# IC3Net/IC3Net

Hardware: NVIDIA H100
Metric: agent-env-steps/sec (higher is better)
Workload: dtype f32

## Files before the change

ic3net_b200/_lib.py:

```python
import ctypes as C
import os

import torch

_HERE = os.path.dirname(os.path.abspath(__file__))
LIB_PATH = os.path.join(_HERE, "libic3net_b200.so")

MAX_AGENTS = 32
MAX_HEADS = 4
MAX_HEAD_DIM = 16
MAX_PASSES = 4
CELL_LSTM, CELL_TANH = 0, 1
LSTM_IMG_BYTES = 786432

ERR_EPISODE_DONE = 1
ERR_ROUTE_OVERRUN = 2
ERR_BAD_ACTION = 4
ERR_PIPELINE = 0x100
ERR_FP16_RANGE = 0x200

PP_MODES = {"mixed": 0, "cooperative": 1, "competitive": 2}

_p = C.c_void_p


class PPCfg(C.Structure):
    _fields_ = [("B", C.c_int32), ("N", C.c_int32), ("dim", C.c_int32), ("vision", C.c_int32),
                ("mode", C.c_int32), ("naction", C.c_int32), ("env_id0", C.c_uint32), ("enemy_comm", C.c_int32),
                ("seed", C.c_uint64)]


class PPState(C.Structure):
    _fields_ = [("loc", _p), ("reached", _p), ("done", _p), ("success", _p), ("episode", _p), ("tick", _p)]


class RolloutIO(C.Structure):
    _fields_ = [("t", C.c_int32), ("max_steps", C.c_int32), ("nheads", C.c_int32), ("hard_attn", C.c_int32),
                ("comm_action_one", C.c_int32), ("last", C.c_int32), ("action", _p), ("t_ep", _p), ("fresh", _p),
                ("comm_next", _p), ("alive_next", _p), ("rec_reward", _p), ("rec_episode_mask", _p),
                ("rec_mini_mask", _p), ("rec_alive", _p), ("stat_reward", _p), ("stat_comm", _p),
                ("stat_success", _p), ("stat_episodes", _p), ("stat_steps", _p), ("batch_size", C.c_int32),
                ("reserved0", C.c_int32), ("halted", _p), ("rec_valid", _p), ("snap_T", C.c_int32),
                ("reserved1", C.c_int32), ("snap_fresh", _p), ("snap_comm", _p), ("snap_alive", _p), ("snap_tep", _p),
                ("snap_pp_loc", _p), ("snap_tj_loc", _p), ("snap_tj_alive", _p), ("snap_tj_last_act", _p),
                ("snap_tj_route_id", _p), ("head_partial", _p), ("head_b", _p), ("head_value", _p), ("head_logp", _p),
                ("head_dim", C.c_int32 * MAX_HEADS)]


class TJCfg(C.Structure):
    _fields_ = [("B", C.c_int32), ("N", C.c_int32), ("vision", C.c_int32), ("h", C.c_int32), ("w", C.c_int32),
                ("G", C.c_int32), ("P", C.c_int32), ("Lmax", C.c_int32), ("outside_cls", C.c_int32),
                ("car_cls", C.c_int32), ("vocab", C.c_int32), ("npath", C.c_int32), ("spawn_thr", C.c_uint32),
                ("env_id0", C.c_uint32), ("seed", C.c_uint64), ("grid", _p), ("route_len", _p), ("route_cells", _p)]


class TJState(C.Structure):
    _fields_ = [("loc", _p), ("alive", _p), ("wait", _p), ("route_id", _p), ("route_pos", _p), ("last_act", _p),
                ("completed", _p), ("cars_in_sys", _p), ("has_failed", _p), ("tick", _p)]


class PolicyCfg(C.Structure):
    _fields_ = [("B", C.c_int32), ("N", C.c_int32), ("H", C.c_int32), ("O", C.c_int32), ("nheads", C.c_int32),
                ("head_dim", C.c_int32 * MAX_HEADS), ("hard_attn", C.c_int32), ("comm_avg", C.c_int32),
                ("comm_mask_zero", C.c_int32), ("env_id0", C.c_uint32), ("seed", C.c_uint64),
                ("obs_off", C.c_int32), ("obs_vocab", C.c_int32), ("obs_ncount", C.c_int32), ("cell", C.c_int32),
                ("passes", C.c_int32), ("x_tanh", C.c_int32), ("h_from_x", C.c_int32), ("reserved0", C.c_int32)]


class PolicyParams(C.Structure):
    _fields_ = [("encoder_w", _p), ("encoder_b", _p), ("c_w", _p), ("c_b", _p), ("w_ih", _p), ("w_hh", _p),
                ("b_ih", _p), ("b_hh", _p), ("value_w", _p), ("value_b", _p),
                ("head_w", _p * MAX_HEADS), ("head_b", _p * MAX_HEADS), ("c_w_pass", _p * MAX_PASSES),
                ("c_b_pass", _p * MAX_PASSES), ("f_w_pass", _p * MAX_PASSES), ("f_b_pass", _p * MAX_PASSES)]


class PolicyPacked(C.Structure):
    _fields_ = [("enc_wT", _p), ("enc_b", _p), ("c_wT", _p), ("c_b", _p), ("lstm_wT", _p), ("lstm_b", _p),
                ("head_w", _p), ("head_b", _p), ("lstm_img", _p), ("bias_cat", _p), ("f_wT", _p), ("f_b", _p), ("flags", _p)]


class PolicyIO(C.Structure):
    _fields_ = [("x", _p), ("h", _p), ("c", _p), ("comm_action", _p), ("alive", _p), ("fresh", _p), ("tick", _p),
                ("draws", _p), ("h_out", _p), ("c_out", _p), ("value", _p), ("logp", _p), ("action", _p),
                ("workspace", _p), ("err", _p), ("pp_env", _p), ("pp_state", _p), ("tj_env", _p), ("tj_state", _p),
                ("x_table", _p), ("defer_heads", C.c_int32), ("pass_index", C.c_int32)]


class BpttPlan(C.Structure):
    _fields_ = [("cfg", C.POINTER(PolicyCfg)), ("w", C.POINTER(PolicyPacked)), ("pp_env", C.POINTER(PPCfg)),
                ("tj_env", C.POINTER(TJCfg)), ("x_table", _p), ("value_coeff", C.c_float), ("entr", C.c_float),
                ("workspace", _p)]


class BpttStepIO(C.Structure):
    _fields_ = [("t", C.c_int32), ("reserved0", C.c_int32), ("h_prev", _p), ("c_prev", _p), ("h_new", _p), ("fresh", _p), ("comm", _p), ("alive", _p), ("cut", _p),
                ("pp_loc", _p), ("tj_loc", _p), ("tj_alive", _p), ("tj_last_act", _p), ("tj_route_id", _p),
                ("logp", _p), ("action", _p), ("value", _p), ("ret", _p), ("adv", _p), ("alive_post", _p),
                ("valid", _p), ("dh", _p), ("dc", _p), ("err", _p)]


_PTR = C.c_void_p
SYMBOLS = {
    "ic3_version": (C.c_char_p, []),
    "ic3_strerror": (C.c_char_p, [C.c_int]),
    "ic3_launch_count": (C.c_uint64, []),
    "ic3_pp_reset": (C.c_int, [C.POINTER(PPCfg), C.POINTER(PPState), _PTR, _PTR, _PTR]),
    "ic3_pp_step": (C.c_int, [C.POINTER(PPCfg), C.POINTER(PPState), _PTR, C.c_int32, _PTR, _PTR, _PTR,
                              C.POINTER(RolloutIO), _PTR]),
    "ic3_pp_obs": (C.c_int, [C.POINTER(PPCfg), C.POINTER(PPState), _PTR, _PTR]),
    "ic3_pp_obs_bounded": (C.c_int, [C.POINTER(PPCfg), C.POINTER(PPState), _PTR, _PTR]),
    "ic3_tj_reset": (C.c_int, [C.POINTER(TJCfg), C.POINTER(TJState), _PTR, _PTR, _PTR]),
    "ic3_tj_step": (C.c_int, [C.POINTER(TJCfg), C.POINTER(TJState), _PTR, C.c_int32, _PTR, _PTR, _PTR, _PTR,
                              C.POINTER(RolloutIO), _PTR]),
    "ic3_tj_obs": (C.c_int, [C.POINTER(TJCfg), C.POINTER(TJState), _PTR, _PTR]),
    "ic3_tj_obs_bounded": (C.c_int, [C.POINTER(TJCfg), C.POINTER(TJState), _PTR, _PTR]),
    "ic3_policy_pack": (C.c_int, [C.POINTER(PolicyCfg), C.POINTER(PolicyParams), C.POINTER(PolicyPacked), _PTR]),
    "ic3_encoder_dense": (C.c_int, [C.POINTER(PolicyCfg), C.POINTER(PolicyPacked), _PTR, _PTR, _PTR]),
    "ic3_pp_encoder_index": (C.c_int, [C.POINTER(PPCfg), C.POINTER(PPState), C.POINTER(PolicyCfg),
                                       C.POINTER(PolicyPacked), _PTR, _PTR]),
    "ic3_tj_encoder_index": (C.c_int, [C.POINTER(TJCfg), C.POINTER(TJState), C.POINTER(PolicyCfg),
                                       C.POINTER(PolicyPacked), _PTR, _PTR]),
    "ic3_pp_obs_encode": (C.c_int, [C.POINTER(PPCfg), C.POINTER(PPState), C.POINTER(PolicyCfg),
                                    C.POINTER(PolicyPacked), _PTR, _PTR, _PTR]),
    "ic3_tj_obs_encode": (C.c_int, [C.POINTER(TJCfg), C.POINTER(TJState), C.POINTER(PolicyCfg),
                                    C.POINTER(PolicyPacked), _PTR, _PTR, _PTR]),
    "ic3_pp_encoder_table":(C.c_int, [C.POINTER(PPCfg), C.POINTER(PolicyCfg), C.POINTER(PolicyPacked), _PTR, _PTR]),
    "ic3_tj_encoder_table": (C.c_int, [C.POINTER(TJCfg), C.POINTER(PolicyCfg), C.POINTER(PolicyPacked), _PTR, _PTR]),
    "ic3_policy_workspace_bytes": (C.c_uint64, [C.POINTER(PolicyCfg)]),
    "ic3_policy_step": (C.c_int, [C.POINTER(PolicyCfg), C.POINTER(PolicyPacked), C.POINTER(PolicyIO), _PTR]),
    "ic3_policy_partial_ptr": (C.c_void_p, [C.POINTER(PolicyCfg), _PTR]),
    "ic3_policy_step_profile": (C.c_int, [C.POINTER(PolicyCfg), C.POINTER(PolicyPacked), C.POINTER(PolicyIO), _PTR,
                                          C.POINTER(C.c_float)]),
    "ic3_sample_actions": (C.c_int, [C.POINTER(PolicyCfg), _PTR, _PTR, _PTR, _PTR, _PTR]),
    "ic3_returns_scan": (C.c_int, [C.c_int32, C.c_int32, C.c_int32, C.c_float, C.c_float, _PTR, _PTR, _PTR, _PTR,
                                   _PTR]),
    "ic3_bptt_workspace_bytes": (C.c_uint64, [C.POINTER(BpttPlan)]),
    "ic3_bptt_begin": (C.c_int, [C.POINTER(BpttPlan), C.c_float, _PTR]),
    "ic3_bptt_step": (C.c_int, [C.POINTER(BpttPlan), C.POINTER(BpttStepIO), _PTR]),
    "ic3_bptt_prepare": (C.c_int, [C.POINTER(BpttPlan), C.POINTER(BpttStepIO), _PTR]),
    "ic3_bptt_finish": (C.c_int, [C.POINTER(BpttPlan), C.POINTER(PolicyParams), C.POINTER(PolicyParams), _PTR, _PTR]),
    "ic3_stat_reduce": (C.c_int, [C.c_int32, C.c_int32, _PTR, _PTR, _PTR, _PTR, _PTR, _PTR, _PTR, _PTR]),
    "ic3_rmsprop_step": (C.c_int, [C.c_int64, C.c_float, C.c_float, C.c_float, C.c_float, _PTR, _PTR, _PTR, _PTR]),
}

_lib = None


def load():
    global _lib
    if _lib is not None:
        return _lib
    if not os.path.exists(LIB_PATH):
        raise RuntimeError("ic3net_b200: %s not found; run `python -m ic3net_b200.build` "
                           "(there is no CPU fallback)" % LIB_PATH)
    lib = C.CDLL(LIB_PATH)
    for name, (res, args) in SYMBOLS.items():
        fn = getattr(lib, name)
        fn.restype = res
        fn.argtypes = args
    _lib = lib
    return lib


def check(rc):
    if rc != 0:
        raise RuntimeError("ic3net_b200 call failed (%d): %s" % (rc, load().ic3_strerror(rc).decode()))


def ptr(t):
    if t is None:
        return None
    assert t.is_cuda and t.is_contiguous(), "ic3net_b200 needs contiguous CUDA tensors"
    return t.data_ptr()


_raw_stream = getattr(torch._C, "_cuda_getCurrentRawStream", None)


def stream():
    if _raw_stream is not None:
        return _raw_stream(torch.cuda.current_device())
    return torch.cuda.current_stream().cuda_stream


def require_cuda():
    if not torch.cuda.is_available():
        raise RuntimeError("ic3net_b200 runs on a CUDA device only (no CPU fallback)")
    load()


def launch_count():
    return int(load().ic3_launch_count())
```

ic3net_b200/csrc/policy_tc.cu:

```cuda
#include <algorithm>

#include "policy_tc_kernels.cuh"


constexpr int TC_TILE_PAD = 8;
constexpr size_t LSTM_SMEM_BYTES = NSTAGE_P * STAGE_BYTES + 256 + TC_H * HEAD_PAD * sizeof(float) + 4 * TC_H * sizeof(float);

static int ctas_beside_lstm(const void* kern, int threads, size_t smem, int* per_sm, int* nsm) {
  cudaFuncAttributes la, ka;
  cudaError_t e = cudaFuncGetAttributes(&la, lstm_tc_kernel);
  if (e == cudaSuccess) e = cudaFuncGetAttributes(&ka, kern);
  int dev = 0, regs = 0, smem_sm = 0, reserved = 0, thr_sm = 0, blk_sm = 0;
  if (e == cudaSuccess) e = cudaGetDevice(&dev);
  if (e == cudaSuccess) e = cudaDeviceGetAttribute(nsm, cudaDevAttrMultiProcessorCount, dev);
  if (e == cudaSuccess) e = cudaDeviceGetAttribute(&regs, cudaDevAttrMaxRegistersPerMultiprocessor, dev);
  if (e == cudaSuccess) e = cudaDeviceGetAttribute(&smem_sm, cudaDevAttrMaxSharedMemoryPerMultiprocessor, dev);
  if (e == cudaSuccess) e = cudaDeviceGetAttribute(&reserved, cudaDevAttrReservedSharedMemoryPerBlock, dev);
  if (e == cudaSuccess) e = cudaDeviceGetAttribute(&thr_sm, cudaDevAttrMaxThreadsPerMultiProcessor, dev);
  if (e == cudaSuccess) e = cudaDeviceGetAttribute(&blk_sm, cudaDevAttrMaxBlocksPerMultiprocessor, dev);
  if (e != cudaSuccess) return (int)e;
  auto cta_regs = [](const cudaFuncAttributes& a, int nthr) { return ((a.numRegs * 32 + 255) / 256 * 256) * ((nthr + 31) / 32); };
  const long free_regs = (long)regs - cta_regs(la, TC_P_THREADS);
  const long free_smem = (long)smem_sm - (long)(LSTM_SMEM_BYTES + la.sharedSizeBytes + reserved);
  long n = free_regs / cta_regs(ka, threads);
  n = std::min(n, free_smem / (long)(smem + ka.sharedSizeBytes + reserved));
  n = std::min(n, (long)(thr_sm - TC_P_THREADS) / threads);
  n = std::min(n, (long)blk_sm - 1);
  *per_sm = n > 1 ? (int)n : 1;
  return IC3_OK;
}

int ic3_grid_beside_lstm(const void* kern, int threads, size_t smem, int nwork, int* grid) {
  struct Entry { const void* kern; int threads; size_t smem; int ctas; };
  static Entry cache[8];
  static int ncache = 0;
  int ctas = 0;
  for (int i = 0; i < ncache; ++i)
    if (cache[i].kern == kern && cache[i].threads == threads && cache[i].smem == smem) ctas = cache[i].ctas;
  if (ctas == 0) {
    cudaError_t e = cudaFuncSetAttribute(kern, cudaFuncAttributePreferredSharedMemoryCarveout, cudaSharedmemCarveoutMaxShared);
    if (e != cudaSuccess) return (int)e;
    int per_sm = 0, nsm = 0;
    const int rc = ctas_beside_lstm(kern, threads, smem, &per_sm, &nsm);
    if (rc) return rc;
    ctas = per_sm * nsm;
    if (ncache < 8) cache[ncache++] = Entry{kern, threads, smem, ctas};
  }
  *grid = nwork < ctas ? nwork : ctas;
  return IC3_OK;
}

static int launch_lstm(const ic3_policy_cfg* cfg, const ic3_policy_io* io, const ic3_policy_packed* w, const __half* a_img,
                       int ntiles_pad, size_t smem, int nout, float* partial, cudaStream_t s) {
  static int max_ctas = 0;
  auto kern = lstm_tc_kernel;
  if (max_ctas == 0) {
    cudaError_t e = cudaFuncSetAttribute(kern, cudaFuncAttributeMaxDynamicSharedMemorySize, (int)smem);
    if (e != cudaSuccess) return (int)e;
    int per_sm = 0, dev = 0, nsm = 0;
    e = cudaOccupancyMaxActiveBlocksPerMultiprocessor(&per_sm, kern, TC_P_THREADS, smem);
    if (e == cudaSuccess) e = cudaGetDevice(&dev);
    if (e == cudaSuccess) e = cudaDeviceGetAttribute(&nsm, cudaDevAttrMultiProcessorCount, dev);
    if (e != cudaSuccess || per_sm <= 0) return e != cudaSuccess ? (int)e : IC3_E_RANGE;
    max_ctas = per_sm * nsm;
  }
  const int nitems = 2 * ntiles_pad;
  cudaLaunchConfig_t lc{};
  lc.gridDim = dim3(nitems < max_ctas ? nitems : max_ctas);
  lc.blockDim = dim3(TC_P_THREADS);
  lc.dynamicSmemBytes = smem;
  lc.stream = s;
  cudaLaunchAttribute la[1];
  la[0].id = cudaLaunchAttributeProgrammaticStreamSerialization;
  la[0].val.programmaticStreamSerializationAllowed = 1;
  lc.attrs = la; lc.numAttrs = ic3_pdl_enabled() ? 1 : 0;
  const __half* b_img = reinterpret_cast<const __half*>(w->lstm_img) + (size_t)io->pass_index * B_IMG_HALFS;
  cudaError_t e = cudaLaunchKernelEx(&lc, kern, *cfg, *io, a_img, b_img,
                                     (const float*)w->bias_cat + (size_t)io->pass_index * 4 * TC_H, nitems,
                                     (const float*)w->head_w, nout, partial);
  ++g_ic3_launches;
  return e == cudaSuccess ? IC3_OK : (int)e;
}

uint64_t ic3_tc_workspace_bytes(const ic3_policy_cfg* cfg) {
  if (!cfg || cfg->H != TC_H) return 0;
  const long R = (long)cfg->B * cfg->N;
  const long ntiles = (R + TC_M - 1) / TC_M;
  const long ntiles_pad = (ntiles + TC_TILE_PAD - 1) / TC_TILE_PAD * TC_TILE_PAD;
  const uint64_t carry = cfg->passes > 1 ? (uint64_t)4 * R * TC_H * sizeof(float) : 0;
  return (uint64_t)ntiles_pad * TC_NCHUNK * A_CHUNK_BYTES + (uint64_t)R * NSLOT * HEAD_PAD * sizeof(float) + carry;
}

extern "C" const float* ic3_policy_partial_ptr(const ic3_policy_cfg* cfg, const void* workspace) {
  if (!cfg || !workspace || cfg->H != TC_H) return nullptr;
  int nout = 1;
  for (int k = 0; k < cfg->nheads; ++k) nout += cfg->head_dim[k];
  if (nout > HEAD_PAD) return nullptr;
  const long R = (long)cfg->B * cfg->N;
  const long ntiles = (R + TC_M - 1) / TC_M;
  const long ntiles_pad = (ntiles + TC_TILE_PAD - 1) / TC_TILE_PAD * TC_TILE_PAD;
  return reinterpret_cast<const float*>(reinterpret_cast<const unsigned char*>(workspace) +
                                        (size_t)ntiles_pad * TC_NCHUNK * A_CHUNK_BYTES);
}

int ic3_tc_pack(const ic3_policy_cfg* cfg, const ic3_policy_params* p, const ic3_policy_packed* out, cudaStream_t s) {
  if (cfg->H != TC_H) return IC3_E_UNSUPPORTED;
  const int total = 4 * TC_H * TC_K;
  if (out->flags) {
    cudaError_t e = cudaMemsetAsync(out->flags, 0, sizeof(int32_t), s);
    if (e != cudaSuccess) return (int)e;
  }
  const int P = cfg->passes > 1 ? cfg->passes : 1;
  for (int ps = 0; ps < P; ++ps) {
    ic3_policy_params q = *p;
    if (ps > 0 && p->c_w_pass[ps]) q.c_w = p->c_w_pass[ps];
    if (ps > 0 && p->c_b_pass[ps]) q.c_b = p->c_b_pass[ps];
    pack_tc_kernel<<<(total + 255) / 256, 256, 0, s>>>(q, reinterpret_cast<__half*>(out->lstm_img) + (size_t)ps * B_IMG_HALFS,
                                                       out->bias_cat + (size_t)ps * 4 * TC_H, out->flags);
    IC3_LAUNCH_CHECK();
  }
  return IC3_OK;
}

static cudaEvent_t* g_prof_ev = nullptr;
static inline void prof_mark(int i, cudaStream_t s) {
  if (g_prof_ev) cudaEventRecord(g_prof_ev[i], s);
}

extern "C" int ic3_policy_step_profile(const ic3_policy_cfg* cfg, const ic3_policy_packed* w, const ic3_policy_io* io,
                                       void* stream, float* ms) {
  static cudaEvent_t ev[4];
  static bool made = false;
  if (!ms) return IC3_E_NULL;
  if (!made) {
    for (int i = 0; i < 4; ++i) {
      cudaError_t e = cudaEventCreate(&ev[i]);
      if (e != cudaSuccess) return (int)e;
    }
    made = true;
  }
  g_prof_ev = ev;
  const int rc = ic3_policy_step(cfg, w, io, stream);
  g_prof_ev = nullptr;
  if (rc) return rc;
  cudaError_t e = cudaEventSynchronize(ev[3]);
  if (e != cudaSuccess) return (int)e;
  for (int i = 0; i < 3; ++i) {
    e = cudaEventElapsedTime(&ms[i], ev[i], ev[i + 1]);
    if (e != cudaSuccess) return (int)e;
  }
  return IC3_OK;
}

static int tc_pass(const ic3_policy_cfg* cfg, const ic3_policy_packed* w, const ic3_policy_io* io, cudaStream_t s, bool last);

int ic3_tc_policy_step(const ic3_policy_cfg* cfg, const ic3_policy_packed* w, const ic3_policy_io* io, cudaStream_t s) {
  if (cfg->H != TC_H) return IC3_E_UNSUPPORTED;
  if (!io->workspace || !w->lstm_img || !w->bias_cat) return IC3_E_NULL;
  const int P = cfg->passes > 1 ? cfg->passes : 1;
  if (P == 1) return tc_pass(cfg, w, io, s, true);
  const long R = (long)cfg->B * cfg->N;
  ic3_policy_cfg c1 = *cfg;
  c1.passes = 1;
  float* carry = reinterpret_cast<float*>(reinterpret_cast<unsigned char*>(io->workspace) + ic3_tc_workspace_bytes(&c1));
  const size_t RH = (size_t)R * TC_H;
  for (int ps = 0; ps < P; ++ps) {
    ic3_policy_io q = *io;
    q.pass_index = ps;
    if (ps > 0) {
      q.h = carry + (size_t)((ps - 1) & 1) * 2 * RH;
      q.c = q.h + RH;
    }
    if (ps < P - 1) {
      q.h_out = carry + (size_t)(ps & 1) * 2 * RH;
      q.c_out = q.h_out + RH;
    }
    const int rc = tc_pass(cfg, w, &q, s, ps == P - 1);
    if (rc) return rc;
  }
  return IC3_OK;
}

static int tc_pass(const ic3_policy_cfg* cfg, const ic3_policy_packed* w, const ic3_policy_io* io, cudaStream_t s, bool last) {
  const long R = (long)cfg->B * cfg->N;
  const int ntiles = (int)((R + TC_M - 1) / TC_M);
  const int ntiles_pad = (ntiles + TC_TILE_PAD - 1) / TC_TILE_PAD * TC_TILE_PAD;
  __half* img = reinterpret_cast<__half*>(io->workspace);
  PrepSrc src;
  memset(&src, 0, sizeof(src));
  src.wT = w->enc_wT;
  src.bias = w->enc_b;
  src.split = cfg->obs_vocab > 0;
  src.table = io->x_table;
  src.wflags = w->flags;
  if (src.table && !src.split) return IC3_E_RANGE;
  prof_mark(0, s);
  if (io->x) {
    IC3_LAUNCH_RC(ic3_launch_pdl(prep_kernel<XSRC_TENSOR, false>, dim3(2 * ntiles_pad), dim3(PREP_THREADS), prep_T_bytes(cfg->N), s, *cfg, *io, img, src, PrepBwd{}));
  } else if (io->pp_env && io->pp_state) {
    const int W = 2 * io->pp_env->vision + 1;
    if (W * W > PREP_MAX_WW || io->pp_env->B != cfg->B || ic3_pp_agents(*io->pp_env) != cfg->N) return IC3_E_RANGE;
    if (cfg->O != W * W * (io->pp_env->dim * io->pp_env->dim + 4)) return IC3_E_RANGE;
    src.pp = *io->pp_env;
    src.pps = *io->pp_state;
    if (int lrc = ic3_pp_layout_check(io->pp_env, cfg)) return lrc;
    if (src.table) {
      IC3_LAUNCH_RC(ic3_launch_pdl(prep_kernel<XSRC_PP, true>, dim3(2 * ntiles_pad), dim3(PREP_THREADS), prep_T_bytes(cfg->N), s, *cfg, *io, img, src, PrepBwd{}));
    } else {
      static bool cfgd = false;
      if (!cfgd) {
        cudaError_t e = cudaFuncSetAttribute(prep_kernel<XSRC_PP, false>, cudaFuncAttributeMaxDynamicSharedMemorySize, PREP_X_BYTES + (PREP_ROWS + 2) * TC_H * 4);
        if (e != cudaSuccess) return (int)e;
        cfgd = true;
      }
      IC3_LAUNCH_RC(ic3_launch_pdl(prep_kernel<XSRC_PP, false>, dim3(2 * ntiles_pad), dim3(256), PREP_X_BYTES + prep_T_bytes(cfg->N), s, *cfg, *io, img, src, PrepBwd{}));
    }
  } else if (io->tj_env && io->tj_state) {
    const int W = 2 * io->tj_env->vision + 1;
    if (W * W > PREP_MAX_WW || io->tj_env->B != cfg->B || io->tj_env->N != cfg->N) return IC3_E_RANGE;
    if (cfg->O != 2 + W * W * io->tj_env->vocab) return IC3_E_RANGE;
    src.tj = *io->tj_env;
    src.tjs = *io->tj_state;
    if (int lrc = ic3_tj_layout_check(io->tj_env, cfg)) return lrc;
    if (src.table) {
      IC3_LAUNCH_RC(ic3_launch_pdl(prep_kernel<XSRC_TJ, true>, dim3(2 * ntiles_pad), dim3(PREP_THREADS), prep_T_bytes(cfg->N), s, *cfg, *io, img, src, PrepBwd{}));
    } else {
      static bool cfgd = false;
      if (!cfgd) {
        cudaError_t e = cudaFuncSetAttribute(prep_kernel<XSRC_TJ, false>, cudaFuncAttributeMaxDynamicSharedMemorySize, PREP_X_BYTES + (PREP_ROWS + 2) * TC_H * 4);
        if (e != cudaSuccess) return (int)e;
        cfgd = true;
      }
      IC3_LAUNCH_RC(ic3_launch_pdl(prep_kernel<XSRC_TJ, false>, dim3(2 * ntiles_pad), dim3(256), PREP_X_BYTES + prep_T_bytes(cfg->N), s, *cfg, *io, img, src, PrepBwd{}));
    }
  } else {
    return IC3_E_NULL;
  }
  prof_mark(1, s);
  const size_t smem = LSTM_SMEM_BYTES;
  int nout = 1;
  for (int k = 0; k < cfg->nheads; ++k) nout += cfg->head_dim[k];
  const bool fused_heads = nout <= HEAD_PAD;
  float* partial = fused_heads ? reinterpret_cast<float*>(reinterpret_cast<unsigned char*>(io->workspace) +
                                                           (size_t)ntiles_pad * TC_NCHUNK * A_CHUNK_BYTES)
                               : nullptr;
  const int rc = launch_lstm(cfg, io, w, img, ntiles_pad, smem, nout, partial, s);
  if (rc) return rc;
  prof_mark(2, s);
  if (!last) return IC3_OK;
  if (fused_heads && io->defer_heads) {
    prof_mark(3, s);
    return IC3_OK;
  }
  if (fused_heads) {
    IC3_LAUNCH_RC(ic3_launch_pdl(heads_finish_kernel, dim3((unsigned)((R + 127) / 128)), dim3(128), 0, s, *cfg, *w, *io,
                                 (const float*)partial));
    prof_mark(3, s);
    return IC3_OK;
  }
  const int P = nout <= 8 ? 8 : (nout <= 16 ? 16 : 32);
  const long rows_per_block = 8L * (32 / P);
  const int hgrid = (int)((R + rows_per_block - 1) / rows_per_block);
  if (P == 8) heads_kernel<8><<<hgrid, 256, 0, s>>>(*cfg, *w, *io);
  else if (P == 16) heads_kernel<16><<<hgrid, 256, 0, s>>>(*cfg, *w, *io);
  else heads_kernel<32><<<hgrid, 256, 0, s>>>(*cfg, *w, *io);
  IC3_LAUNCH_CHECK();
  prof_mark(3, s);
  return IC3_OK;
}
```

ic3net_b200/csrc/policy_tc_kernels.cuh:

```cuda
#pragma once
#include <cuda_fp16.h>

#include <cstdlib>
#include <cstring>

#include "ic3_common.cuh"
#include "policy_heads.cuh"
#include "policy_internal.h"
#include "tc_common.cuh"

namespace {

constexpr int TC_H = 128;
constexpr int TC_K = 384;
constexpr int TC_KC = 32;
constexpr int TC_NCHUNK = TC_K / TC_KC;
constexpr int TC_M = 128;
constexpr int TC_NH = 256;
constexpr int A_CHUNK_BYTES = 2 * TC_M * TC_KC * 2;
constexpr int B_CHUNK_BYTES = 2 * TC_NH * TC_KC * 2;
constexpr int STAGE_BYTES = A_CHUNK_BYTES + B_CHUNK_BYTES;
constexpr int A_TILE_HALFS = TC_NCHUNK * A_CHUNK_BYTES / 2;

__host__ __device__ __forceinline__ size_t a_img_off(int tile, int k, int r, int part) {
  return (size_t)tile * A_TILE_HALFS + (size_t)part * (A_TILE_HALFS / 2) + ((size_t)(k >> 3) * 16 + (r >> 3)) * 64 + (r & 7) * 8 +
         (k & 7);
}
__host__ __device__ __forceinline__ size_t b_img_off(int nh, int k, int n, int part) {
  const int c = k >> 5, kk = k & 31;
  return ((((((size_t)(nh * TC_NCHUNK + c) * 2 + part) * 4 + (kk >> 3)) * 32 + (n >> 3)) * 8 + (n & 7)) * 8) + (kk & 7);
}

constexpr size_t B_IMG_HALFS = (size_t)2 * TC_NCHUNK * B_CHUNK_BYTES / 2;

__global__ void pack_tc_kernel(ic3_policy_params p, __half* __restrict__ img, float* __restrict__ bias_cat,
                               int32_t* __restrict__ flags) {
  const int H = TC_H;
  const int idx = blockIdx.x * blockDim.x + threadIdx.x;
  if (idx < 4 * H * TC_K) {
    const int col = idx / TC_K, k = idx - col * TC_K;
    const int u = col >> 2, g = col & 3, row = g * H + u;
    double w;
    if (k < H) {
      w = p.w_ih[(size_t)row * H + k];
    } else if (k < 2 * H) {
      double acc = 0.0;
      for (int m = 0; m < H; ++m) acc += (double)p.w_ih[(size_t)row * H + m] * (double)p.c_w[(size_t)m * H + (k - H)];
      w = acc;
    } else {
      w = p.w_hh[(size_t)row * H + (k - 2 * H)];
    }
    __half hi, lo;
    split_f16((float)w, SCALE_B, hi, lo);
    if (flags && !(fabs(w) * SCALE_B < 65504.0)) atomicOr(flags, IC3_ERR_FP16_RANGE);
    const int nh = col >> 8, n = col & 255;
    img[b_img_off(nh, k, n, 0)] = hi;
    img[b_img_off(nh, k, n, 1)] = lo;
  }
  if (idx < 4 * H) {
    const int u = idx >> 2, g = idx & 3, row = g * H + u;
    double acc = (double)p.b_ih[row] + (double)p.b_hh[row];
    for (int m = 0; m < H; ++m) acc += (double)p.w_ih[(size_t)row * H + m] * (double)p.c_b[m];
    bias_cat[idx] = (float)acc;
  }
}

constexpr int PREP_ROWS = 64;
constexpr int PREP_THREADS = 160;
__host__ __device__ inline size_t prep_T_bytes(int N) { return (size_t)(PREP_ROWS / N + 2) * TC_H * sizeof(float); }
constexpr int PREP_MAX_WW = 25;
constexpr int PREP_X_BYTES = PREP_ROWS * TC_H * 4;

enum { XSRC_TENSOR = 0, XSRC_PP = 1, XSRC_TJ = 2 };
struct PrepSrc {
  ic3_pp_cfg pp;
  ic3_pp_state pps;
  ic3_tj_cfg tj;
  ic3_tj_state tjs;
  const float* wT;
  const float* bias;
  const float* table;
  int split;
  const int32_t* wflags;
};

__device__ __forceinline__ void fma4(float4& a, float v, const float4 w) {
  a.x = fmaf(v, w.x, a.x); a.y = fmaf(v, w.y, a.y); a.z = fmaf(v, w.z, a.z); a.w = fmaf(v, w.w, a.w);
}

__device__ __forceinline__ void fma4_sel(bool sel, float4& a, float4& b, float v, const float4 w) {
  if (sel) fma4(a, v, w);
  else fma4(b, v, w);
}

struct PrepBwd {
  __half* p_img;
  float* gs;
  float* gr;
  int npg;
  int npos;
};

template <int XSRC, bool TAB, bool BWD = false>
__global__ void __launch_bounds__(256) prep_kernel(ic3_policy_cfg cfg, ic3_policy_io io, __half* __restrict__ img,
                                                   PrepSrc src, PrepBwd bw) {
  static_assert(!(TAB && XSRC == XSRC_TENSOR), "the table belongs to the fused index encoder");
  static_assert(!BWD || TAB, "the backward pass uses the per-position table form of the encoder");
  __shared__ float s_gate[PREP_ROWS + 64];
  __shared__ float s_den[PREP_ROWS + 64];
  __shared__ int s_feat[(XSRC == XSRC_TENSOR || TAB) ? 1 : PREP_ROWS * PREP_MAX_WW];
  __shared__ int s_cnt[XSRC == XSRC_TENSOR ? 1 : PREP_ROWS * PREP_MAX_WW];
  __shared__ unsigned s_mask[TAB ? PREP_ROWS : 1];
  __shared__ int s_pos[TAB ? PREP_ROWS : 1];
  __shared__ float s_la[XSRC == XSRC_TJ ? PREP_ROWS : 1], s_ri[XSRC == XSRC_TJ ? PREP_ROWS : 1];
  __shared__ int s_live[XSRC == XSRC_TJ ? PREP_ROWS : 1];
  extern __shared__ __align__(16) float s_dyn[];
  float (*s_T)[TC_H] = reinterpret_cast<float (*)[TC_H]>(s_dyn);
  float* s_x = s_dyn + (size_t)(PREP_ROWS / cfg.N + 2) * TC_H;
  const int N = cfg.N;
  const int R = cfg.B * N;
  const int tile = blockIdx.x >> 1, hb = blockIdx.x & 1;
  const int row0 = tile * TC_M + hb * PREP_ROWS;
  ic3_pdl_trigger();
  if (TAB) {
    if (threadIdx.x < PREP_ROWS) s_mask[threadIdx.x] = 0u;
    __syncthreads();
  }
  ic3_pdl_wait();
  if (blockIdx.x == 0 && threadIdx.x == 0 && src.wflags && io.err && *src.wflags) atomicOr(io.err, *src.wflags);
  for (int w = threadIdx.x; w < PREP_ROWS + 64; w += blockDim.x) {
    const int row = row0 - 32 + w;
    float g = 0.f, den = 1.f;
    if (row >= 0 && row < R) {
      const int e = row / N, i = row - e * N;
      const bool fr = io.fresh && io.fresh[e];
      int n_alive = N, al = 1;
      if (io.alive && !fr) {
        n_alive = 0;
        for (int j = 0; j < N; ++j) n_alive += io.alive[(size_t)e * N + j] != 0;
        al = io.alive[(size_t)e * N + i] != 0;
      }
      int cm = 1;
      if (cfg.hard_attn) cm = fr ? 0 : (io.comm_action[(size_t)e * N + i] != 0);
      g = (fr && io.pass_index == 0) ? 0.f : (float)(al * cm);
      if (cfg.comm_avg && n_alive > 1) den = (float)(n_alive - 1);
    }
    s_gate[w] = g;
    s_den[w] = den;
  }
  if (XSRC == XSRC_PP) {
    const int D = src.pp.dim, v = src.pp.vision, W = 2 * v + 1, WW = W * W, V = D * D + 4;
    const int NP = src.pp.N;
    for (int p = threadIdx.x; p < PREP_ROWS * WW; p += blockDim.x) {
      const int rl = p / WW, w = p - rl * WW, row = row0 + rl;
      int feat = 0, cnt = 0;
      if (row < R) {
        const int e = row / N, i = row - e * N;
        const int* l = src.pps.loc + (size_t)e * (NP + 1) * 2;
        const int dy = w / W, dx = w - dy * W;
        const int rr = l[2 * i] - v + dy, cc = l[2 * i + 1] - v + dx;
        if (rr >= 0 && rr < D && cc >= 0 && cc < D) {
          int npred = 0;
          for (int j = 0; j < NP; ++j) npred += (l[2 * j] == rr && l[2 * j + 1] == cc);
          const int nprey = (l[2 * NP] == rr && l[2 * NP + 1] == cc);
          feat = w * V + rr * D + cc;
          cnt = npred | (nprey << 8);
        } else {
          feat = w * V + V - 3;
        }
        if (TAB && w == 0) s_pos[rl] = l[2 * i] * D + l[2 * i + 1];
      } else if (TAB && w == 0) {
        s_pos[rl] = -1;
      }
      if (!TAB) s_feat[rl * WW + w] = feat;
      s_cnt[rl * WW + w] = cnt;
      if (TAB && cnt) atomicOr(&s_mask[rl], 1u << w);
    }
  } else if (XSRC == XSRC_TJ) {
    const int v = src.tj.vision, W = 2 * v + 1, WW = W * W, V = src.tj.vocab;
    for (int rl = threadIdx.x; rl < PREP_ROWS; rl += blockDim.x) {
      const int row = row0 + rl;
      int live = 0;
      float la = 0.f, ri = 0.f;
      if (row < R) {
        live = src.tjs.alive[row] != 0;
        la = (float)src.tjs.last_act[row];
        ri = (float)src.tjs.route_id[row] / (float)(src.tj.npath - 1);
      }
      s_live[rl] = live; s_la[rl] = la; s_ri[rl] = ri;
    }
    for (int p = threadIdx.x; p < PREP_ROWS * WW; p += blockDim.x) {
      const int rl = p / WW, w = p - rl * WW, row = row0 + rl;
      int feat = 0, cnt = 0;
      if (row < R) {
        const int e = row / N;
        const int* l = src.tjs.loc + (size_t)e * N * 2;
        const int i = row - e * N;
        const int dy = w / W, dx = w - dy * W;
        const int rr = l[2 * i] - v + dy, cc = l[2 * i + 1] - v + dx;
        int cls = src.tj.outside_cls;
        if (rr >= 0 && rr < src.tj.h && cc >= 0 && cc < src.tj.w) {
          cls = src.tj.grid[rr * src.tj.w + cc];
          for (int j = 0; j < N; ++j) cnt += (l[2 * j] == rr && l[2 * j + 1] == cc);
        }
        feat = 2 + w * V + cls;
        if (TAB && w == 0) s_pos[rl] = src.tjs.alive[row] ? l[2 * i] * src.tj.w + l[2 * i + 1] : -1;
        if (TAB && !src.tjs.alive[row]) cnt = 0;
      } else if (TAB && w == 0) {
        s_pos[rl] = -1;
      }
      if (!TAB) s_feat[rl * WW + w] = feat;
      s_cnt[rl * WW + w] = cnt;
      if (TAB && cnt) atomicOr(&s_mask[rl], 1u << w);
    }
  }
  __syncthreads();
  if (XSRC != XSRC_TENSOR && !TAB) {
    const int gw = threadIdx.x >> 5, gl = threadIdx.x & 31;
    const float4* wq = reinterpret_cast<const float4*>(src.wT) + gl;
    const bool split = src.split != 0;
    for (int rl = gw; rl < PREP_ROWS; rl += (blockDim.x >> 5)) {
      float4 xv = __ldg(reinterpret_cast<const float4*>(src.bias) + gl);
      float4 x2 = make_float4(0.f, 0.f, 0.f, 0.f);
      const int row = row0 + rl;
      if (row < R) {
        if (XSRC == XSRC_PP) {
          const int W = 2 * src.pp.vision + 1, WW = W * W, V = src.pp.dim * src.pp.dim + 4;
          for (int w = 0; w < WW; ++w) {
            const int feat = s_feat[rl * WW + w], cnt = s_cnt[rl * WW + w];
            fma4(xv, 1.f, __ldg(wq + (size_t)feat * (TC_H / 4)));
            if (cnt >> 8) fma4_sel(split, x2, xv, (float)(cnt >> 8), __ldg(wq + (size_t)(w * V + V - 2) * (TC_H / 4)));
            if (cnt & 255) fma4_sel(split, x2, xv, (float)(cnt & 255), __ldg(wq + (size_t)(w * V + V - 1) * (TC_H / 4)));
          }
        } else if (s_live[rl]) {
          const int W = 2 * src.tj.vision + 1, WW = W * W, V = src.tj.vocab;
          if (s_la[rl] != 0.f) fma4_sel(split, x2, xv, s_la[rl], __ldg(wq));
          if (s_ri[rl] != 0.f) fma4_sel(split, x2, xv, s_ri[rl], __ldg(wq + (TC_H / 4)));
          for (int w = 0; w < WW; ++w) {
            const int feat = s_feat[rl * WW + w], cnt = s_cnt[rl * WW + w];
            fma4(xv, 1.f, __ldg(wq + (size_t)feat * (TC_H / 4)));
            if (cnt) fma4_sel(split, x2, xv, (float)cnt, __ldg(wq + (size_t)(2 + w * V + src.tj.car_cls) * (TC_H / 4)));
          }
        }
      }
      xv.x += x2.x; xv.y += x2.y; xv.z += x2.z; xv.w += x2.w;
      *reinterpret_cast<float4*>(&s_x[rl * TC_H + 4 * gl]) = xv;
    }
  }
  const int e_first = row0 / N;
  const int last_row = min(R, row0 + PREP_ROWS) - 1;
  const bool want_s = !cfg.comm_mask_zero && N >= 2 && last_row >= row0;
  if (want_s) {
    const int nenv = last_row / N - e_first + 1;
    for (int idx = threadIdx.x; idx < nenv * (TC_H / 4); idx += blockDim.x) {
      const int el = idx >> 5, q = idx & 31;
      const int base = (e_first + el) * N;
      float4 t = make_float4(0.f, 0.f, 0.f, 0.f);
      for (int j = 0; j < N; ++j) {
        if (s_gate[base + j - row0 + 32] != 0.f) {
          const float4 o = __ldg(reinterpret_cast<const float4*>(io.h + (size_t)(base + j) * TC_H) + q);
          t.x += o.x; t.y += o.y; t.z += o.z; t.w += o.w;
        }
      }
      *reinterpret_cast<float4*>(&s_T[el][4 * q]) = t;
    }
  }
  __syncthreads();
  const int warp = threadIdx.x >> 5, lane = threadIdx.x & 31;
  if (BWD) {
    for (int rl = threadIdx.x; rl < PREP_ROWS; rl += blockDim.x) {
      const int row = row0 + rl;
      if (row < R) {
        bw.gs[row] = s_gate[rl + 32] / s_den[rl + 32];
        bw.gr[row] = s_gate[rl + 32];
      }
    }
    const int WW = XSRC == XSRC_PP ? (2 * src.pp.vision + 1) * (2 * src.pp.vision + 1)
                                   : (2 * src.tj.vision + 1) * (2 * src.tj.vision + 1);
    const int r8 = lane >> 2, c2 = (lane & 3) * 2;
    for (int cm = warp; cm < bw.npg * 8; cm += (blockDim.x >> 5)) {
      const int pg = cm >> 3, rgl = cm & 7;
      const int rl = rgl * 8 + r8, row = row0 + rl;
      float v[2] = {0.f, 0.f};
      if (row < R) {
        const int pos = s_pos[rl];
#pragma unroll
        for (int j = 0; j < 2; ++j) {
          const int col = pg * 8 + c2 + j;
          if (col < bw.npos) {
            v[j] = (col == pos) ? 1.f : 0.f;
          } else {
            const int idx = col - bw.npos;
            if (XSRC == XSRC_PP) {
              if (idx < 2 * WW) {
                const int cnt = s_cnt[rl * WW + (idx >> 1)];
                v[j] = (float)((idx & 1) ? (cnt & 255) : (cnt >> 8));
              } else if (idx == 2 * WW) {
                v[j] = 1.f;
              }
            } else if (XSRC == XSRC_TJ) {
              if (idx < WW) v[j] = pos >= 0 ? (float)s_cnt[rl * WW + idx] : 0.f;
              else if (idx == WW) v[j] = pos >= 0 ? s_la[rl] : 0.f;
              else if (idx == WW + 1) v[j] = pos >= 0 ? __half2float(__float2half_rn(s_ri[rl])) : 0.f;
              else if (idx == WW + 2) v[j] = pos >= 0 ? s_ri[rl] - __half2float(__float2half_rn(s_ri[rl])) : 0.f;
              else if (idx == WW + 3) v[j] = 1.f;
            }
          }
        }
      }
      const size_t off = (((size_t)tile * bw.npg + pg) * 16 + (hb * 8 + rgl)) * 64 + r8 * 8 + c2;
      *reinterpret_cast<__half2*>(bw.p_img + off) = __floats2half2_rn(v[0], v[1]);
    }
  }
  const float4 zero4 = make_float4(0.f, 0.f, 0.f, 0.f);
  const size_t tile_base = (size_t)tile * A_TILE_HALFS;
#pragma unroll 2
  for (int item = warp; item < 64; item += (blockDim.x >> 5)) {
    const int rcl = item & 7, qg = item >> 3;
    const int r8 = lane & 7, q = qg * 4 + (lane >> 3);
    const int rl = rcl * 8 + r8;
    const int rc = hb * 8 + rcl;
    const int row = row0 + rl;
    float4 xv = zero4, hv = zero4, sv = zero4;
    if (row < R) {
      const int e = row / N;
      const bool fr = io.fresh && io.fresh[e] && io.pass_index == 0;
      if (XSRC == XSRC_TENSOR) {
        xv = __ldg(reinterpret_cast<const float4*>(io.x + (size_t)row * TC_H) + q);
      } else if (!TAB) {
        xv = *reinterpret_cast<const float4*>(&s_x[rl * TC_H + 4 * q]);
      } else {
        const int pos = s_pos[rl];
        xv = __ldg(reinterpret_cast<const float4*>(pos >= 0 ? src.table + (size_t)pos * TC_H : src.bias) + q);
        float4 x2 = zero4;
        const float4* wq = reinterpret_cast<const float4*>(src.wT) + q;
        if (XSRC == XSRC_PP) {
          const int W = 2 * src.pp.vision + 1, WW = W * W, V = src.pp.dim * src.pp.dim + 4;
          for (unsigned m = s_mask[rl]; m; m &= m - 1) {
            const int w = __ffs(m) - 1, cnt = s_cnt[rl * WW + w];
            if (cnt >> 8) fma4(x2, (float)(cnt >> 8), __ldg(wq + (size_t)(w * V + V - 2) * (TC_H / 4)));
            if (cnt & 255) fma4(x2, (float)(cnt & 255), __ldg(wq + (size_t)(w * V + V - 1) * (TC_H / 4)));
          }
        } else if (pos >= 0) {
          const int W = 2 * src.tj.vision + 1, WW = W * W, V = src.tj.vocab;
          if (s_la[rl] != 0.f) fma4(x2, s_la[rl], __ldg(wq));
          if (s_ri[rl] != 0.f) fma4(x2, s_ri[rl], __ldg(wq + (TC_H / 4)));
          for (unsigned m = s_mask[rl]; m; m &= m - 1) {
            const int w = __ffs(m) - 1;
            fma4(x2, (float)s_cnt[rl * WW + w], __ldg(wq + (size_t)(2 + w * V + src.tj.car_cls) * (TC_H / 4)));
          }
        }
        xv.x += x2.x; xv.y += x2.y; xv.z += x2.z; xv.w += x2.w;
      }
      if (!fr) hv = __ldg(reinterpret_cast<const float4*>(io.h + (size_t)row * TC_H) + q);
      if (want_s && s_gate[rl + 32] != 0.f) {
        const float4 t = *reinterpret_cast<const float4*>(&s_T[e - e_first][4 * q]);
        const float inv = 1.f / s_den[rl + 32];
        sv.x = (t.x - hv.x) * inv; sv.y = (t.y - hv.y) * inv; sv.z = (t.z - hv.z) * inv; sv.w = (t.w - hv.w) * inv;
      }
    }
    {
      const float m = fmaxf(fmaxf(fmaxf(fabsf(xv.x), fabsf(xv.y)), fmaxf(fabsf(xv.z), fabsf(xv.w))),
                            fmaxf(fmaxf(fmaxf(fabsf(hv.x), fabsf(hv.y)), fmaxf(fabsf(hv.z), fabsf(hv.w))),
                                  fmaxf(fmaxf(fabsf(sv.x), fabsf(sv.y)), fmaxf(fabsf(sv.z), fabsf(sv.w)))));
      if (!(m * SCALE_A < 65504.f) && io.err) atomicOr(io.err, IC3_ERR_FP16_RANGE);
    }
    const size_t cell = tile_base + (size_t)(((q >> 1) * 16 + rc) * 64 + r8 * 8 + (q & 1) * 4);
    constexpr size_t LO = A_TILE_HALFS / 2, SEC = 16 * 1024;
    store_split4(img, cell + 0 * SEC, cell + 0 * SEC + LO, xv, SCALE_A);
    store_split4(img, cell + 1 * SEC, cell + 1 * SEC + LO, sv, SCALE_A);
    store_split4(img, cell + 2 * SEC, cell + 2 * SEC + LO, hv, SCALE_A);
  }
}

__device__ __forceinline__ float ex2_fast(float x) {
  float y;
  asm("ex2.approx.ftz.f32 %0, %1;" : "=f"(y) : "f"(x));
  return y;
}
__device__ __forceinline__ float rcp_fast(float x) {
  float y;
  asm("rcp.approx.ftz.f32 %0, %1;" : "=f"(y) : "f"(x));
  return y;
}
constexpr float LOG2E = 1.4426950408889634f;

__device__ __forceinline__ void load_scaled_bias(float* s_bias, const float* __restrict__ bias_cat) {
  for (int idx = threadIdx.x; idx < 4 * TC_H; idx += blockDim.x)
    s_bias[idx] = __ldg(bias_cat + idx) * ((idx & 3) == 2 ? -2.f * LOG2E : -LOG2E);
}

__device__ __forceinline__ void lstm_cell4(const float (&v)[16], const float (&co)[4], const float* s_bias4, int bstride,
                                           float (&cn)[4], float (&hn)[4]) {
  constexpr float SG = -INV_SCALE * LOG2E;
  constexpr float TMAX = 30.f;
  float go[4], bc[4];
#pragma unroll
  for (int j = 0; j < 4; ++j) {
    const float4 b = *reinterpret_cast<const float4*>(s_bias4 + j * bstride);
    const float ai = 1.f + ex2_fast(fminf(fmaf(v[4 * j + 0], SG, b.x), TMAX));
    const float af = 1.f + ex2_fast(fminf(fmaf(v[4 * j + 1], SG, b.y), TMAX));
    const float ag = 1.f + ex2_fast(fminf(fmaf(v[4 * j + 2], 2.f * SG, b.z), TMAX));
    const float ao = 1.f + ex2_fast(fminf(fmaf(v[4 * j + 3], SG, b.w), TMAX));
    const float p1 = ai * af, p2 = ag * ao;
    const float r = rcp_fast(p1 * p2);
    const float r1 = r * p2, r2 = r * p1;
    const float gi = r1 * af, gf = r1 * ai;
    const float gg = fmaf(2.f, r2 * ao, -1.f);
    go[j] = r2 * ag;
    cn[j] = fmaf(gf, co[j], gi * gg);
    bc[j] = 1.f + ex2_fast(fminf(cn[j] * (-2.f * LOG2E), TMAX));
  }
  const float q1 = bc[0] * bc[1], q2 = bc[2] * bc[3];
  const float r = rcp_fast(q1 * q2);
  const float r1 = r * q2, r2 = r * q1;
  hn[0] = go[0] * fmaf(2.f, r1 * bc[1], -1.f);
  hn[1] = go[1] * fmaf(2.f, r1 * bc[0], -1.f);
  hn[2] = go[2] * fmaf(2.f, r2 * bc[3], -1.f);
  hn[3] = go[3] * fmaf(2.f, r2 * bc[2], -1.f);
}

constexpr int NSTAGE_P = 4;
constexpr int HEAD_PAD = IC3_HEAD_PAD;
constexpr int MMA_WARPS = 8;
constexpr int TC_P_THREADS = MMA_WARPS * 32 + 32;
constexpr int NSLOT = IC3_HEAD_NSLOT;

template <int NCHUNK>
__device__ __forceinline__ void wg_gemm_item(float (&d)[128], uint32_t smem_base, uint32_t a_row, uint32_t bar_full,
                                             uint32_t bar_empty, uint32_t li, int lane, bool& ok, int32_t* err) {
  static_assert(NCHUNK % NSTAGE_P == 0, "stage index must be a function of the chunk index alone");
  const uint64_t dA = make_desc(smem_base + a_row, 2048, 128), dB = make_desc(smem_base + A_CHUNK_BYTES, 4096, 128);
  wgmma_fence_regs(d);
#pragma unroll
  for (int c = 0; c < NCHUNK; ++c) {
    const uint32_t s = c % NSTAGE_P;
    if (ok) ok = mbar_wait(bar_full + 8 * s, (li * (NCHUNK / NSTAGE_P) + c / NSTAGE_P) & 1, err);
    wgmma_fence();
#pragma unroll
    for (int ks = 0; ks < TC_KC / 16; ++ks) {
      const uint64_t da_hi = dA + ((s * STAGE_BYTES + ks * 4096) >> 4);
      const uint64_t da_lo = dA + ((s * STAGE_BYTES + A_CHUNK_BYTES / 2 + ks * 4096) >> 4);
      const uint64_t db_hi = dB + ((s * STAGE_BYTES + ks * 8192) >> 4);
      const uint64_t db_lo = dB + ((s * STAGE_BYTES + B_CHUNK_BYTES / 2 + ks * 8192) >> 4);
      wgmma_m64n256_kk(d, da_hi, db_hi, (c | ks) != 0);
      wgmma_m64n256_kk(d, da_lo, db_hi, 1);
      wgmma_m64n256_kk(d, da_hi, db_lo, 1);
    }
    wgmma_commit();
    wgmma_wait<1>();
    if (c > 0) {
      __syncwarp();
      if (lane == 0) mbar_arrive(bar_empty + 8 * ((c - 1) % NSTAGE_P));
    }
  }
  wgmma_wait<0>();
  wgmma_fence_regs(d);
  __syncwarp();
  if (lane == 0) mbar_arrive(bar_empty + 8 * ((NCHUNK - 1) % NSTAGE_P));
}

template <int NCHUNK, typename ASrc, typename BSrc>
__device__ __forceinline__ void ring_producer(uint32_t smem_base, uint32_t bar_full, uint32_t bar_empty, int item0,
                                              int nitems, int stride, size_t a_lo_off, ASrc a_src, BSrc b_src,
                                              int32_t* err) {
  uint32_t li = 0;
  bool ok = true;
  for (int item = item0; item < nitems && ok; item += stride, ++li) {
#pragma unroll
    for (int c = 0; c < NCHUNK; ++c) {
      if (!ok) break;
      const uint32_t s = c % NSTAGE_P;
      ok = mbar_wait(bar_empty + 8 * s, ((li * (NCHUNK / NSTAGE_P) + c / NSTAGE_P) & 1) ^ 1, err);
      const uint32_t dst = smem_base + s * STAGE_BYTES;
      const unsigned char* a = a_src(item, c);
      mbar_expect_tx(bar_full + 8 * s, STAGE_BYTES);
      bulk_g2s(dst, a, A_CHUNK_BYTES / 2, bar_full + 8 * s);
      bulk_g2s(dst + A_CHUNK_BYTES / 2, a + a_lo_off, A_CHUNK_BYTES / 2, bar_full + 8 * s);
      bulk_g2s(dst + A_CHUNK_BYTES, b_src(item, c), B_CHUNK_BYTES, bar_full + 8 * s);
    }
  }
}

__device__ __forceinline__ void gather_gates(const float (&d)[128], int j, bool odd, float (&g)[4]) {
  const float s0 = odd ? d[4 * j + 0] : d[4 * j + 2];
  const float s1 = odd ? d[4 * j + 1] : d[4 * j + 3];
  const float r0 = __shfl_xor_sync(IC3_FULL_MASK, s0, 1), r1 = __shfl_xor_sync(IC3_FULL_MASK, s1, 1);
  g[0] = odd ? r0 : d[4 * j + 0];
  g[1] = odd ? r1 : d[4 * j + 1];
  g[2] = odd ? d[4 * j + 2] : r0;
  g[3] = odd ? d[4 * j + 3] : r1;
}

__device__ __forceinline__ void pair_store2(float* rowp, int j, bool hi_lane, float a, float b, bool st) {
  const float r = __shfl_xor_sync(IC3_FULL_MASK, hi_lane ? a : b, 2);
  const float2 v = hi_lane ? make_float2(r, b) : make_float2(a, r);
  if (st) *reinterpret_cast<float2*>(rowp + 2 * j + (hi_lane ? 2 : 0)) = v;
}
__device__ __forceinline__ void pair_load2(const float* rowp, int j, bool hi_lane, bool ld, float& a, float& b) {
  const float2 v = ld ? *reinterpret_cast<const float2*>(rowp + 2 * j + (hi_lane ? 2 : 0)) : make_float2(0.f, 0.f);
  const float r = __shfl_xor_sync(IC3_FULL_MASK, hi_lane ? v.x : v.y, 2);
  a = hi_lane ? r : v.x;
  b = hi_lane ? v.y : r;
}

__device__ __forceinline__ void epilogue_item(const ic3_policy_cfg& cfg, const ic3_policy_io& io, const float* s_bias,
                                              const float* s_hw, float* __restrict__ partial, const float (&d)[128],
                                              int tile, int nh, int wg, int w4, int lane, bool ok) {
  const int R = cfg.B * cfg.N;
  const bool odd = lane & 1, hl = (lane >> 1) & 1;
  const int row = tile * TC_M + wg * 64 + w4 * 16 + (lane >> 2) + (odd ? 8 : 0);
  const bool st = ok && row < R;
  bool fr = false;
  if (row < R && io.fresh && io.pass_index == 0) fr = io.fresh[row / cfg.N] != 0;
  const int ub = nh * (TC_NH / 4) + hl;
  const float* crow = io.c + (size_t)row * TC_H + nh * (TC_NH / 4);
  float part[2][HEAD_PAD];
#pragma unroll
  for (int h = 0; h < 2; ++h)
#pragma unroll
    for (int o = 0; o < HEAD_PAD; ++o) part[h][o] = 0.f;
#pragma unroll
  for (int j0 = 0; j0 < 32; j0 += 4) {
    float v[16], co[4], cn[4], hn[4];
    pair_load2(crow, j0, hl, row < R && !fr, co[0], co[1]);
    pair_load2(crow, j0 + 2, hl, row < R && !fr, co[2], co[3]);
#pragma unroll
    for (int jj = 0; jj < 4; ++jj) {
      float g[4];
      gather_gates(d, j0 + jj, odd, g);
      v[4 * jj + 0] = g[0]; v[4 * jj + 1] = g[1]; v[4 * jj + 2] = g[2]; v[4 * jj + 3] = g[3];
    }
    lstm_cell4(v, co, s_bias + 4 * (ub + 2 * j0), 8, cn, hn);
    if (partial) {
#pragma unroll
      for (int jj = 0; jj < 4; ++jj) {
        const int u = ub + 2 * (j0 + jj);
        const float4 w0 = *reinterpret_cast<const float4*>(&s_hw[u * HEAD_PAD]);
        const float4 w1 = *reinterpret_cast<const float4*>(&s_hw[u * HEAD_PAD + 4]);
        float* p = part[j0 >= 16];
        p[0] = fmaf(hn[jj], w0.x, p[0]); p[1] = fmaf(hn[jj], w0.y, p[1]);
        p[2] = fmaf(hn[jj], w0.z, p[2]); p[3] = fmaf(hn[jj], w0.w, p[3]);
        p[4] = fmaf(hn[jj], w1.x, p[4]); p[5] = fmaf(hn[jj], w1.y, p[5]);
        p[6] = fmaf(hn[jj], w1.z, p[6]); p[7] = fmaf(hn[jj], w1.w, p[7]);
      }
    }
    float* co_row = io.c_out + (size_t)row * TC_H + nh * (TC_NH / 4);
    float* ho_row = io.h_out + (size_t)row * TC_H + nh * (TC_NH / 4);
#pragma unroll
    for (int pr = 0; pr < 2; ++pr) {
      pair_store2(co_row, j0 + 2 * pr, hl, cn[2 * pr], cn[2 * pr + 1], st);
      pair_store2(ho_row, j0 + 2 * pr, hl, hn[2 * pr], hn[2 * pr + 1], st);
    }
  }
  if (partial && st) {
    float4* p = reinterpret_cast<float4*>(partial + ((size_t)row * NSLOT + nh * 4 + hl * 2) * HEAD_PAD);
    p[0] = make_float4(part[0][0], part[0][1], part[0][2], part[0][3]);
    p[1] = make_float4(part[0][4], part[0][5], part[0][6], part[0][7]);
    p[2] = make_float4(part[1][0], part[1][1], part[1][2], part[1][3]);
    p[3] = make_float4(part[1][4], part[1][5], part[1][6], part[1][7]);
  }
}

__global__ void __launch_bounds__(TC_P_THREADS, 1) lstm_tc_kernel(ic3_policy_cfg cfg, ic3_policy_io io,
                                                                 const __half* __restrict__ a_img,
                                                                 const __half* __restrict__ b_img,
                                                                 const float* __restrict__ bias_cat, int nitems,
                                                                 const float* __restrict__ head_w, int nout,
                                                                 float* __restrict__ partial) {
  extern __shared__ __align__(1024) unsigned char smem[];
  uint64_t* bars = reinterpret_cast<uint64_t*>(smem + NSTAGE_P * STAGE_BYTES);
  float* s_hw = reinterpret_cast<float*>(smem + NSTAGE_P * STAGE_BYTES + 256);
  float* s_bias = s_hw + TC_H * HEAD_PAD;
  ic3_pdl_trigger();
  const uint32_t bar_full = smem_u32(bars), bar_empty = smem_u32(bars + NSTAGE_P);
  const int warp = threadIdx.x >> 5, lane = threadIdx.x & 31;
  if (threadIdx.x == 0) {
    for (int s = 0; s < NSTAGE_P; ++s) {
      mbar_init(bar_full + 8 * s, 1);
      mbar_init(bar_empty + 8 * s, MMA_WARPS);
    }
    asm volatile("fence.mbarrier_init.release.cluster;" ::: "memory");
  }
  ic3_pdl_wait();
  load_scaled_bias(s_bias, bias_cat);
  if (partial) {
    for (int idx = threadIdx.x; idx < TC_H * HEAD_PAD; idx += blockDim.x) {
      const int u = idx / HEAD_PAD, o = idx - u * HEAD_PAD;
      s_hw[idx] = o < nout ? __ldg(head_w + (size_t)o * TC_H + u) : 0.f;
    }
  }
  __syncthreads();
  const uint32_t smem_base = smem_u32(smem);

  if (warp == MMA_WARPS) {
    if (lane == 0) {
      const unsigned char* a = reinterpret_cast<const unsigned char*>(a_img);
      const unsigned char* b = reinterpret_cast<const unsigned char*>(b_img);
      ring_producer<TC_NCHUNK>(
          smem_base, bar_full, bar_empty, blockIdx.x, nitems, gridDim.x, (size_t)A_TILE_HALFS,
          [=](int item, int c) { return a + (size_t)(item >> 1) * TC_NCHUNK * A_CHUNK_BYTES + (size_t)c * (A_CHUNK_BYTES / 2); },
          [=](int item, int c) { return b + (size_t)((item & 1) * TC_NCHUNK + c) * B_CHUNK_BYTES; }, io.err);
    }
  } else {
    const int wg = warp >> 2, w4 = warp & 3;
    float d[128];
#pragma unroll
    for (int i = 0; i < 128; ++i) d[i] = 0.f;
    uint32_t li = 0;
    bool ok = true;
    for (int item = blockIdx.x; item < nitems; item += gridDim.x, ++li) {
      wg_gemm_item<TC_NCHUNK>(d, smem_base, wg * 1024, bar_full, bar_empty, li, lane, ok, io.err);
      epilogue_item(cfg, io, s_bias, s_hw, partial, d, item >> 1, item & 1, wg, w4, lane, ok);
    }
  }
}

template <int P>
__global__ void __launch_bounds__(256) heads_kernel(ic3_policy_cfg cfg, ic3_policy_packed w, ic3_policy_io io) {
  constexpr int RPW = 32 / P;
  const int lane = threadIdx.x & 31, o = lane % P;
  const long R = (long)cfg.B * cfg.N;
  const long row = ((long)blockIdx.x * (blockDim.x >> 5) + (threadIdx.x >> 5)) * RPW + lane / P;
  const bool live = row < R;
  int atot = 0;
  for (int k = 0; k < cfg.nheads; ++k) atot += cfg.head_dim[k];
  const int nout = 1 + atot;
  __shared__ float s_w[TC_H * P];
  for (int idx = threadIdx.x; idx < TC_H * P; idx += blockDim.x) {
    const int k = idx / P, oo = idx - k * P;
    s_w[idx] = oo < nout ? __ldg(w.head_w + (size_t)oo * TC_H + k) : 0.f;
  }
  __syncthreads();
  float logit = 0.f;
  if (live) {
    const float4* hp = reinterpret_cast<const float4*>(io.h_out + (size_t)row * TC_H);
    float a0 = 0.f, a1 = 0.f, a2 = 0.f, a3 = 0.f;
#pragma unroll 8
    for (int q = 0; q < TC_H / 4; ++q) {
      const float4 hv = hp[q];
      a0 = fmaf(hv.x, s_w[(4 * q + 0) * P + o], a0);
      a1 = fmaf(hv.y, s_w[(4 * q + 1) * P + o], a1);
      a2 = fmaf(hv.z, s_w[(4 * q + 2) * P + o], a2);
      a3 = fmaf(hv.w, s_w[(4 * q + 3) * P + o], a3);
    }
    logit = (a0 + a1) + (a2 + a3) + (o < nout ? __ldg(w.head_b + o) : 0.f);
  }
  if (live && o == 0) io.value[row] = logit;
  const bool do_sample = io.action != nullptr;
  const int e = live ? (int)(row / cfg.N) : 0, i = live ? (int)(row - (long)e * cfg.N) : 0;
  uint32_t w0 = 0, w1 = 0, w2 = 0, w3 = 0;
  if (do_sample && !io.draws) {
    if (o == 0 && live) {
      const uint4 d = ic3_draw24(cfg.seed, cfg.env_id0 + (uint32_t)e, io.tick ? io.tick[e] : 0u, IC3_STREAM_ACTION, (uint32_t)i);
      w0 = d.x; w1 = d.y; w2 = d.z; w3 = d.w;
    }
    w0 = __shfl_sync(IC3_FULL_MASK, w0, 0, P); w1 = __shfl_sync(IC3_FULL_MASK, w1, 0, P);
    w2 = __shfl_sync(IC3_FULL_MASK, w2, 0, P); w3 = __shfl_sync(IC3_FULL_MASK, w3, 0, P);
  }
  int off = 1;
  for (int k = 0; k < cfg.nheads; ++k) {
    const int na = cfg.head_dim[k];
    float m = -INFINITY;
    for (int a = 0; a < na; ++a) m = fmaxf(m, __shfl_sync(IC3_FULL_MASK, logit, off + a, P));
    float s = 0.f;
    for (int a = 0; a < na; ++a) s += expf(__shfl_sync(IC3_FULL_MASK, logit, off + a, P) - m);
    const float mylogp = logit - (m + logf(s));
    uint32_t u24 = 0;
    if (do_sample) {
      if (io.draws) u24 = live ? io.draws[(size_t)row * cfg.nheads + k] : 0u;
      else u24 = k == 0 ? w0 : (k == 1 ? w1 : (k == 2 ? w2 : w3));
    }
    const float u = (float)u24 * 5.9604644775390625e-08f;
    int act = na - 1;
    if (do_sample) {
      float cdf = 0.f;
      bool found = false;
      for (int a = 0; a < na; ++a) {
        cdf += expf(__shfl_sync(IC3_FULL_MASK, mylogp, off + a, P));
        if (!found && cdf > u) {
          act = a;
          found = true;
        }
      }
    }
    if (live && o >= off && o < off + na) io.logp[(size_t)row * atot + (off - 1) + (o - off)] = mylogp;
    if (live && do_sample && o == 0) io.action[(size_t)row * cfg.nheads + k] = act;
    off += na;
  }
}

__global__ void __launch_bounds__(128) heads_finish_kernel(ic3_policy_cfg cfg, ic3_policy_packed w, ic3_policy_io io,
                                                            const float* __restrict__ partial) {
  ic3_pdl_trigger();
  ic3_pdl_wait();
  const long row = (long)blockIdx.x * blockDim.x + threadIdx.x;
  if (row >= (long)cfg.B * cfg.N) return;
  HeadsFinish f;
  f.partial = partial; f.head_b = w.head_b; f.nheads = cfg.nheads;
#pragma unroll
  for (int k = 0; k < IC3_MAX_HEADS; ++k) f.head_dim[k] = cfg.head_dim[k];
  f.seed = cfg.seed; f.env_id0 = cfg.env_id0; f.tick = io.tick; f.draws = io.draws;
  f.value = io.value; f.logp = io.logp; f.action = io.action;
  const int e = (int)(row / cfg.N), i = (int)(row - (long)e * cfg.N);
  heads_finish_row(f, row, e, i, nullptr);
}

}
```

ic3net_b200/csrc/pp_env.cu:

```cuda
#include <cstring>

#include "encoder_rows.cuh"
#include "ic3_common.cuh"
#include "policy_internal.h"
#include "rollout_tail.cuh"

namespace {

struct PPArgs {
  ic3_pp_cfg cfg;
  ic3_pp_state st;
};

__device__ __forceinline__ void pp_reset_env(const PPArgs& a, int e, int lane) {
  const int N = a.cfg.N, D = a.cfg.dim, need = N + 1;
  const uint32_t ncell = (uint32_t)(D * D);
  const uint32_t epi = a.st.episode[e];
  int mycell = -1, cnt = 0;
  for (uint32_t blk = 0; cnt < need && blk < 4096u; ++blk) {
    const uint4 w = ic3_draw24(a.cfg.seed, a.cfg.env_id0 + (uint32_t)e, epi, IC3_STREAM_PP_RESET, blk);
#pragma unroll
    for (int i = 0; i < 4; ++i) {
      if (cnt < need) {
        const int cand = (int)ic3_pick(ic3_word(w, i), ncell);
        const bool dup = __any_sync(IC3_FULL_MASK, lane < cnt && mycell == cand);
        if (!dup) {
          if (lane == cnt) mycell = cand;
          ++cnt;
        }
      }
    }
  }
  if (lane < need) {
    int* l = a.st.loc + ((size_t)e * need + lane) * 2;
    l[0] = mycell / D;
    l[1] = mycell % D;
  }
  if (lane < N) a.st.reached[(size_t)e * N + lane] = 0;
  if (lane == 0) {
    a.st.episode[e] = epi + 1;
    a.st.done[e] = 0;
    a.st.success[e] = -1;
  }
}

__global__ void pp_reset_kernel(PPArgs a, const uint8_t* __restrict__ mask) {
  const int e = blockIdx.x * (blockDim.x >> 5) + (threadIdx.x >> 5);
  if (e >= a.cfg.B) return;
  if (mask && !mask[e]) return;
  pp_reset_env(a, e, threadIdx.x & 31);
}

template <bool VEC4>
__device__ __forceinline__ void pp_write_obs(const ic3_pp_cfg& cfg, const int* s_r, const int* s_c,
                                            uint32_t* s_cell, float* __restrict__ obs_env, bool keep) {
  const int N = cfg.N, D = cfg.dim, v = cfg.vision, W = 2 * v + 1, WW = W * W;
  const int V = D * D + 4, OUTSIDE = D * D + 1;
  const int ncell = ic3_pp_agents(cfg) * WW;
  for (int c = threadIdx.x; c < ncell; c += blockDim.x) {
    const int i = c / WW, w = c - i * WW, dy = w / W, dx = w - dy * W;
    const int rr = s_r[i] - v + dy, cc = s_c[i] - v + dx;
    uint32_t info = (uint32_t)OUTSIDE;
    if (rr >= 0 && rr < D && cc >= 0 && cc < D) {
      int npred = 0;
      for (int j = 0; j < N; ++j) npred += (s_r[j] == rr && s_c[j] == cc);
      const int nprey = (s_r[N] == rr && s_c[N] == cc);
      info = (uint32_t)(rr * D + cc) | ((uint32_t)npred << 16) | ((uint32_t)nprey << 24);
    }
    s_cell[c] = info;
  }
  __syncthreads();
  const int warp = threadIdx.x >> 5, lane = threadIdx.x & 31, nwarp = blockDim.x >> 5;
  for (int c = warp; c < ncell; c += nwarp) {
    const uint32_t info = s_cell[c];
    const int cls = (int)(info & 0xffffu);
    const float npred = (float)((info >> 16) & 0xffu), nprey = (float)(info >> 24);
    float* dst = obs_env + (size_t)c * V;
    if (VEC4) {
      const int V4 = V >> 2, qc = cls >> 2, qp = (V - 1) >> 2, qy = (V - 2) >> 2;
      for (int q = lane; q < V4; q += 32) {
        float4 o = make_float4(0.f, 0.f, 0.f, 0.f);
        if (q == qc) {
          const int k = cls & 3;
          o.x = k == 0 ? 1.f : 0.f; o.y = k == 1 ? 1.f : 0.f; o.z = k == 2 ? 1.f : 0.f; o.w = k == 3 ? 1.f : 0.f;
        }
        if (q == qy) {
          o.z = nprey;
        }
        if (q == qp) {
          o.w = npred;
        }
        ic3_st_obs(reinterpret_cast<float4*>(dst) + q, o, keep);
      }
    } else {
      for (int q = lane; q < V; q += 32) {
        float o = (q == cls) ? 1.f : 0.f;
        if (q == V - 2) o = nprey;
        if (q == V - 1) o = npred;
        ic3_st_obs(dst + q, o, keep);
      }
    }
  }
}

template <bool VEC4>
__global__ void pp_step_kernel(PPArgs a, const int32_t* __restrict__ act, int act_stride,
                               float* __restrict__ reward, float* __restrict__ obs, int32_t* err,
                               RolloutOpt r, int do_step, int keep_l2) {
  ic3_pdl_trigger();
  ic3_pdl_wait();
  extern __shared__ uint32_t s_cell[];
  __shared__ int s_r[IC3_MAX_AGENTS + 1], s_c[IC3_MAX_AGENTS + 1];
  const int N = a.cfg.N, D = a.cfg.dim;
  const int NA = ic3_pp_agents(a.cfg);
  const int warp = threadIdx.x >> 5, lane = threadIdx.x & 31;
  const int e = obs ? (int)blockIdx.x : (int)(blockIdx.x * (blockDim.x >> 5)) + warp;
  if (obs ? warp == 0 : e < a.cfg.B) {
    int rr = 0, cc = 0, rch = 0;
    if (lane <= N) {
      const int* l = a.st.loc + ((size_t)e * (N + 1) + lane) * 2;
      rr = l[0];
      cc = l[1];
    }
    if (lane < N) rch = a.st.reached[(size_t)e * N + lane];
    if (do_step && r.has && ic3_rollout_halted(r.io, e, a.cfg.B, NA, lane)) {
    } else if (do_step) {
      if (a.st.done[e]) {
        if (lane == 0) atomicOr(err, IC3_ERR_EPISODE_DONE);
      } else {
        int av = 4;
        if (r.has && r.io.head_partial) av = ic3_rollout_heads(r.io, a.cfg.seed, a.cfg.env_id0, a.st.tick, e, NA, lane);
        else if (lane < NA) av = act[((size_t)e * NA + lane) * act_stride];
        if (lane >= NA) av = 4;
        if (lane < NA && (av < 0 || av > a.cfg.naction)) atomicOr(err, IC3_ERR_BAD_ACTION);
        if (lane < N && !rch) {
          if (av == 0) rr = max(0, rr - 1);
          else if (av == 1) cc = min(D - 1, cc + 1);
          else if (av == 2) rr = min(D - 1, rr + 1);
          else if (av == 3) cc = max(0, cc - 1);
        }
        const int pr = __shfl_sync(IC3_FULL_MASK, rr, N), pc = __shfl_sync(IC3_FULL_MASK, cc, N);
        const bool on = lane < N && rr == pr && cc == pc;
        const int n_on = __popc(__ballot_sync(IC3_FULL_MASK, on));
        double rew = -0.05;
        if (on) {
          if (a.cfg.mode == IC3_PP_COOPERATIVE) rew = 0.05 * (double)n_on;
          else if (a.cfg.mode == IC3_PP_COMPETITIVE) rew = 0.05 / (double)n_on;
          else rew = 0.0;
        }
        if (lane == N) rew = n_on == 0 ? 0.05 : 0.0;
        rch |= on ? 1 : 0;
        const bool allr = __ballot_sync(IC3_FULL_MASK, lane >= N || rch) == IC3_FULL_MASK;
        const bool done = (a.cfg.mode == IC3_PP_MIXED) && allr;
        int success = a.st.success[e];
        if (a.cfg.mode != IC3_PP_COMPETITIVE) success = (n_on == N) ? 1 : 0;
        if (lane < N) {
          int* l = a.st.loc + ((size_t)e * (N + 1) + lane) * 2;
          l[0] = rr;
          l[1] = cc;
          a.st.reached[(size_t)e * N + lane] = (uint8_t)rch;
        }
        if (lane < NA) reward[(size_t)e * NA + lane] = (float)rew;
        if (lane == 0) {
          a.st.done[e] = done ? 1 : 0;
          a.st.success[e] = success;
          a.st.tick[e] += 1;
        }
        if (r.has) {
          const bool done_t = ic3_rollout_tail(r.io, e, a.cfg.B, NA, lane, (float)rew, done, 1, 0, success);
          if (done_t) {
            __syncwarp();
            pp_reset_env(a, e, lane);
            __syncwarp();
            if (lane <= N) {
              const int* l = a.st.loc + ((size_t)e * (N + 1) + lane) * 2;
              rr = l[0];
              cc = l[1];
            }
          }
        }
      }
    }
    if (do_step && r.has && r.io.snap_T > 0) {
      __syncwarp();
      ic3_rollout_snapshot(r.io, e, a.cfg.B, NA, lane);
      if (r.io.snap_pp_loc && r.io.t + 1 < r.io.snap_T && lane <= N) {
        int* d = r.io.snap_pp_loc + (((size_t)(r.io.t + 1) * a.cfg.B + e) * (N + 1) + lane) * 2;
        d[0] = rr;
        d[1] = cc;
      }
    }
    if (obs && lane <= N) {
      s_r[lane] = rr;
      s_c[lane] = cc;
    }
  }
  if (obs == nullptr) return;
  __syncthreads();
  const int W = 2 * a.cfg.vision + 1;
  pp_write_obs<VEC4>(a.cfg, s_r, s_c, s_cell, obs + (size_t)e * NA * W * W * (D * D + 4), keep_l2 != 0);
}

template <int H, bool VEC4>
__global__ void __launch_bounds__(256) pp_obs_encode_kernel(PPArgs a, float* __restrict__ obs,
                                                            const float* __restrict__ wT, const float* __restrict__ bias,
                                                            float* __restrict__ x, bool split, int keep_l2) {
  ic3_pdl_trigger();
  ic3_pdl_wait();
  extern __shared__ uint32_t s_cell[];
  __shared__ int s_r[IC3_MAX_AGENTS + 1], s_c[IC3_MAX_AGENTS + 1];
  const int N = a.cfg.N, D = a.cfg.dim, W = 2 * a.cfg.vision + 1, WW = W * W, V = D * D + 4;
  const int NA = ic3_pp_agents(a.cfg);
  const int e = blockIdx.x, warp = threadIdx.x >> 5, lane = threadIdx.x & 31;
  if (threadIdx.x <= N) {
    const int* l = a.st.loc + ((size_t)e * (N + 1) + threadIdx.x) * 2;
    s_r[threadIdx.x] = l[0];
    s_c[threadIdx.x] = l[1];
  }
  __syncthreads();
  pp_write_obs<VEC4>(a.cfg, s_r, s_c, s_cell, obs + (size_t)e * NA * WW * V, keep_l2 != 0);
  for (int i = warp; i < NA; i += blockDim.x >> 5) {
    const uint32_t* rec = s_cell + i * WW;
    pp_encode_row<H>([rec](int w) { return rec[w]; }, WW, V, wT, bias, split, x + ((size_t)e * NA + i) * H, lane);
  }
}

template <bool VEC4>
__global__ void __launch_bounds__(IC3_OBS_WRITER_THREADS, IC3_OBS_WRITER_MIN_CTAS)
    pp_obs_writer_kernel(PPArgs a, float* __restrict__ obs, int keep_l2) {
  ic3_pdl_trigger();
  ic3_pdl_wait();
  extern __shared__ uint32_t s_cell[];
  __shared__ int s_r[IC3_MAX_AGENTS + 1], s_c[IC3_MAX_AGENTS + 1];
  const int N = a.cfg.N, W = 2 * a.cfg.vision + 1, B = a.cfg.B;
  const size_t per_env = (size_t)ic3_pp_agents(a.cfg) * W * W * (a.cfg.dim * a.cfg.dim + 4);
  const int k = threadIdx.x;
  int r = 0, c = 0;
  if (k <= N && (int)blockIdx.x < B) {
    const int* l = a.st.loc + ((size_t)blockIdx.x * (N + 1) + k) * 2;
    r = l[0];
    c = l[1];
  }
  for (int e = blockIdx.x; e < B; e += gridDim.x) {
    if (k <= N) {
      s_r[k] = r;
      s_c[k] = c;
      if (e + (int)gridDim.x < B) {
        const int* l = a.st.loc + ((size_t)(e + gridDim.x) * (N + 1) + k) * 2;
        r = l[0];
        c = l[1];
      }
    }
    __syncthreads();
    pp_write_obs<VEC4>(a.cfg, s_r, s_c, s_cell, obs + (size_t)e * per_env, keep_l2 != 0);
    __syncthreads();
  }
}

int pp_check(const ic3_pp_cfg* cfg, const ic3_pp_state* st) {
  if (!cfg || !st) return IC3_E_NULL;
  if (!st->loc || !st->reached || !st->done || !st->success || !st->episode || !st->tick) return IC3_E_NULL;
  if (cfg->B <= 0 || cfg->N <= 0 || cfg->N >= IC3_MAX_AGENTS) return IC3_E_RANGE;
  if (cfg->dim <= 0 || cfg->dim > 181 || cfg->vision < 0 || cfg->vision > 7) return IC3_E_RANGE;
  if (cfg->N + 1 > cfg->dim * cfg->dim) return IC3_E_RANGE;
  if (cfg->mode < 0 || cfg->mode > 2) return IC3_E_RANGE;
  if (cfg->naction != 4 && cfg->naction != 5) return IC3_E_RANGE;
  return IC3_OK;
}

int pp_launch(const ic3_pp_cfg* cfg, const ic3_pp_state* st, const int32_t* act, int act_stride,
              float* reward, float* obs, int32_t* err, const ic3_rollout_io* r, int do_step,
              cudaStream_t s) {
  PPArgs a{*cfg, *st};
  const int W = 2 * cfg->vision + 1;
  const int V = cfg->dim * cfg->dim + 4;
  const int NA = ic3_pp_agents(*cfg);
  const size_t smem = obs ? (size_t)NA * W * W * sizeof(uint32_t) : 0;
  const int threads = obs ? 256 : 32 * IC3_ENV_WARPS;
  const int grid = obs ? cfg->B : (cfg->B + IC3_ENV_WARPS - 1) / IC3_ENV_WARPS;
  const bool vec4 = (V % 4 == 0) && ((reinterpret_cast<uintptr_t>(obs) & 15) == 0);
  RolloutOpt ro = make_rollout_opt(r);
  const int keep = obs && (size_t)cfg->B * NA * W * W * V * sizeof(float) <= IC3_OBS_L2_KEEP_BYTES;
  if (vec4)
    IC3_LAUNCH_RC(ic3_launch_pdl(pp_step_kernel<true>, dim3(grid), dim3(threads), smem, s, a, act, act_stride, reward, obs,
                                 err, ro, do_step, keep));
  else
    IC3_LAUNCH_RC(ic3_launch_pdl(pp_step_kernel<false>, dim3(grid), dim3(threads), smem, s, a, act, act_stride, reward, obs,
                                 err, ro, do_step, keep));
  return IC3_OK;
}

template <int H>
int pp_obs_encode_launch(const ic3_pp_cfg* cfg, const ic3_pp_state* st, const ic3_policy_cfg* pcfg,
                         const ic3_policy_packed* w, float* obs, float* x, cudaStream_t s) {
  PPArgs a{*cfg, *st};
  const int W = 2 * cfg->vision + 1, V = cfg->dim * cfg->dim + 4, NA = ic3_pp_agents(*cfg);
  const size_t smem = (size_t)NA * W * W * sizeof(uint32_t);
  const bool vec4 = (V % 4 == 0) && ((reinterpret_cast<uintptr_t>(obs) & 15) == 0);
  const bool split = pcfg->obs_vocab > 0;
  const int keep = (size_t)cfg->B * NA * W * W * V * sizeof(float) <= IC3_OBS_L2_KEEP_BYTES;
  const float* wT = w->enc_wT;
  const float* b = w->enc_b;
  if (vec4)
    IC3_LAUNCH_RC(ic3_launch_pdl(pp_obs_encode_kernel<H, true>, dim3(cfg->B), dim3(256), smem, s, a, obs, wT, b, x, split,
                                 keep));
  else
    IC3_LAUNCH_RC(ic3_launch_pdl(pp_obs_encode_kernel<H, false>, dim3(cfg->B), dim3(256), smem, s, a, obs, wT, b, x, split,
                                 keep));
  return IC3_OK;
}

template <bool VEC4>
int pp_obs_bounded_launch(const ic3_pp_cfg* cfg, const ic3_pp_state* st, float* obs, cudaStream_t s) {
  PPArgs a{*cfg, *st};
  const int W = 2 * cfg->vision + 1, V = cfg->dim * cfg->dim + 4, NA = ic3_pp_agents(*cfg);
  const size_t smem = (size_t)NA * W * W * sizeof(uint32_t);
  const int keep = (size_t)cfg->B * NA * W * W * V * sizeof(float) <= IC3_OBS_L2_KEEP_BYTES;
  auto kern = pp_obs_writer_kernel<VEC4>;
  int grid = 0;
  const int rc = ic3_grid_beside_lstm((const void*)kern, IC3_OBS_WRITER_THREADS, smem, cfg->B, &grid);
  if (rc) return rc;
  IC3_LAUNCH_RC(ic3_launch_pdl(kern, dim3(grid), dim3(IC3_OBS_WRITER_THREADS), smem, s, a, obs, keep));
  return IC3_OK;
}

}

extern "C" int ic3_pp_obs_bounded(const ic3_pp_cfg* cfg, const ic3_pp_state* st, float* obs, void* stream) {
  int rc = pp_check(cfg, st);
  if (rc) return rc;
  if (!obs) return IC3_E_NULL;
  const bool vec4 = ((cfg->dim * cfg->dim + 4) % 4 == 0) && ((reinterpret_cast<uintptr_t>(obs) & 15) == 0);
  return vec4 ? pp_obs_bounded_launch<true>(cfg, st, obs, (cudaStream_t)stream)
              : pp_obs_bounded_launch<false>(cfg, st, obs, (cudaStream_t)stream);
}

extern "C" int ic3_pp_reset(const ic3_pp_cfg* cfg, const ic3_pp_state* st, const uint8_t* mask,
                            float* obs, void* stream) {
  int rc = pp_check(cfg, st);
  if (rc) return rc;
  cudaStream_t s = (cudaStream_t)stream;
  PPArgs a{*cfg, *st};
  const int wpb = 4;
  pp_reset_kernel<<<(cfg->B + wpb - 1) / wpb, wpb * 32, 0, s>>>(a, mask);
  IC3_LAUNCH_CHECK();
  if (obs) return pp_launch(cfg, st, nullptr, 0, nullptr, obs, nullptr, nullptr, 0, s);
  return IC3_OK;
}

extern "C" int ic3_pp_step(const ic3_pp_cfg* cfg, const ic3_pp_state* st, const int32_t* act,
                           int32_t act_stride, float* reward, float* obs, int32_t* err,
                           const ic3_rollout_io* r, void* stream) {
  int rc = pp_check(cfg, st);
  if (rc) return rc;
  if (!act || !reward || !err || act_stride < 1) return IC3_E_NULL;
  if (r && (!r->t_ep || !r->fresh || !r->alive_next || (r->hard_attn && (!r->comm_next || !r->action))))
    return IC3_E_NULL;
  return pp_launch(cfg, st, act, act_stride, reward, obs, err, r, 1, (cudaStream_t)stream);
}

extern "C" int ic3_pp_obs(const ic3_pp_cfg* cfg, const ic3_pp_state* st, float* obs, void* stream) {
  int rc = pp_check(cfg, st);
  if (rc) return rc;
  if (!obs) return IC3_E_NULL;
  return pp_launch(cfg, st, nullptr, 0, nullptr, obs, nullptr, nullptr, 0, (cudaStream_t)stream);
}

extern "C" int ic3_pp_obs_encode(const ic3_pp_cfg* env, const ic3_pp_state* st, const ic3_policy_cfg* cfg,
                                 const ic3_policy_packed* w, float* obs, float* x, void* stream) {
  int rc = pp_check(env, st);
  if (rc) return rc;
  rc = ic3_encoder_check(cfg, w);
  if (rc) return rc;
  if (!obs || !x) return IC3_E_NULL;
  if (env->B != cfg->B || ic3_pp_agents(*env) != cfg->N) return IC3_E_RANGE;
  const int W = 2 * env->vision + 1;
  if (cfg->O != W * W * (env->dim * env->dim + 4)) return IC3_E_RANGE;
  rc = ic3_pp_layout_check(env, cfg);
  if (rc) return rc;
  IC3_DISPATCH_H(cfg->H, pp_obs_encode_launch<HH>(env, st, cfg, w, obs, x, (cudaStream_t)stream));
}
```

ic3net_b200/csrc/tj_env.cu:

```cuda
#include <cstring>

#include "encoder_rows.cuh"
#include "ic3_common.cuh"
#include "policy_internal.h"
#include "rollout_tail.cuh"

namespace {

struct TJArgs {
  ic3_tj_cfg cfg;
  ic3_tj_state st;
};

__device__ __forceinline__ void tj_reset_env(const TJArgs& a, int e, int lane) {
  const int N = a.cfg.N;
  if (lane < N) {
    const size_t i = (size_t)e * N + lane;
    a.st.loc[i * 2] = 0;
    a.st.loc[i * 2 + 1] = 0;
    a.st.alive[i] = 0;
    a.st.wait[i] = 0;
    a.st.route_id[i] = -1;
    a.st.route_pos[i] = -1;
    a.st.last_act[i] = 0;
    a.st.completed[i] = 0;
  }
  if (lane == 0) {
    a.st.cars_in_sys[e] = 0;
    a.st.has_failed[e] = 0;
  }
}

__global__ void tj_reset_kernel(TJArgs a, const uint8_t* __restrict__ mask) {
  const int e = blockIdx.x * (blockDim.x >> 5) + (threadIdx.x >> 5);
  if (e >= a.cfg.B) return;
  if (mask && !mask[e]) return;
  tj_reset_env(a, e, threadIdx.x & 31);
}

__device__ __forceinline__ void tj_write_obs(const ic3_tj_cfg& cfg, const int* s_r, const int* s_c,
                                            const int* s_alive, const int* s_rid, const int* s_lact,
                                            uint32_t* s_cell, float* __restrict__ obs_env, bool keep) {
  const int N = cfg.N, v = cfg.vision, W = 2 * v + 1, WW = W * W, V = cfg.vocab;
  const int O = 2 + WW * V;
  const int ncell = N * WW;
  for (int c = threadIdx.x; c < ncell; c += blockDim.x) {
    const int i = c / WW, w = c - i * WW, dy = w / W, dx = w - dy * W;
    const int rr = s_r[i] - v + dy, cc = s_c[i] - v + dx;
    uint32_t info = (uint32_t)cfg.outside_cls;
    if (rr >= 0 && rr < cfg.h && cc >= 0 && cc < cfg.w) {
      int cnt = 0;
      for (int j = 0; j < N; ++j) cnt += (s_r[j] == rr && s_c[j] == cc);
      info = (uint32_t)cfg.grid[rr * cfg.w + cc] | ((uint32_t)cnt << 16);
    }
    s_cell[c] = info;
  }
  __syncthreads();
  const int warp = threadIdx.x >> 5, lane = threadIdx.x & 31, nwarp = blockDim.x >> 5;
  for (int c = warp; c < ncell; c += nwarp) {
    const int i = c / WW, w = c - i * WW;
    const uint32_t info = s_cell[c];
    const int cls = (int)(info & 0xffffu);
    const float cnt = (float)(info >> 16);
    const bool live = s_alive[i] != 0;
    float* dst = obs_env + (size_t)i * O + 2 + (size_t)w * V;
    for (int q = lane; q < V; q += 32) {
      float o = (q == cls) ? 1.f : 0.f;
      if (q == cfg.car_cls) o += cnt;
      ic3_st_obs(dst + q, live ? o : 0.f, keep);
    }
  }
  for (int i = threadIdx.x; i < N; i += blockDim.x) {
    const bool live = s_alive[i] != 0;
    float* dst = obs_env + (size_t)i * O;
    dst[0] = live ? (float)s_lact[i] : 0.f;
    dst[1] = live ? (float)s_rid[i] / (float)(cfg.npath - 1) : 0.f;
  }
}

__global__ void tj_step_kernel(TJArgs a, const int32_t* __restrict__ act, int act_stride,
                               const uint32_t* __restrict__ draws, float* __restrict__ reward,
                               float* __restrict__ obs, int32_t* err, RolloutOpt r, int do_step, int keep_l2) {
  ic3_pdl_trigger();
  ic3_pdl_wait();
  extern __shared__ uint32_t s_cell[];
  __shared__ int s_r[IC3_MAX_AGENTS], s_c[IC3_MAX_AGENTS], s_alive[IC3_MAX_AGENTS], s_rid[IC3_MAX_AGENTS],
      s_lact[IC3_MAX_AGENTS];
  const ic3_tj_cfg& cfg = a.cfg;
  const int N = cfg.N;
  const int warp = threadIdx.x >> 5, lane = threadIdx.x & 31;
  const int e = obs ? (int)blockIdx.x : (int)(blockIdx.x * (blockDim.x >> 5)) + warp;
  if (obs ? warp == 0 : e < cfg.B) {
    const size_t i = (size_t)e * N + lane;
    int rr = 0, cc = 0, alive = 0, wait = 0, rid = -1, rpos = -1, lact = 0;
    if (lane < N) {
      rr = a.st.loc[i * 2];
      cc = a.st.loc[i * 2 + 1];
      alive = a.st.alive[i];
      wait = a.st.wait[i];
      rid = a.st.route_id[i];
      rpos = a.st.route_pos[i];
      lact = a.st.last_act[i];
    }
    if (do_step && r.has && ic3_rollout_halted(r.io, e, cfg.B, N, lane)) {
    } else if (do_step) {
      int completed = 0;
      int av = 1;
      if (r.has && r.io.head_partial) av = ic3_rollout_heads(r.io, cfg.seed, cfg.env_id0, a.st.tick, e, N, lane);
      else if (lane < N) av = act[i * act_stride];
      if (lane >= N) av = 1;
      if (lane < N && (av < 0 || av > 2)) atomicOr(err, IC3_ERR_BAD_ACTION);
      if (lane < N && alive) {
        wait += 1;
        if (av == 1) {
          lact = 1;
        } else if (av == 0) {
          rpos += 1;
          const int len = cfg.route_len[rid];
          if (rpos == len) {
            alive = 0;
            wait = 0;
            rr = 0;
            cc = 0;
            completed = 1;
          } else if (rpos > len) {
            atomicOr(err, IC3_ERR_ROUTE_OVERRUN);
          } else {
            const int cell = cfg.route_cells[(size_t)rid * cfg.Lmax + rpos];
            rr = cell >> 16;
            cc = cell & 0xffff;
            lact = 0;
          }
        }
      }
      int cars = a.st.cars_in_sys[e] - __popc(__ballot_sync(IC3_FULL_MASK, completed));
      const uint32_t tick = a.st.tick[e];
      for (int g = 0; g < cfg.G; ++g) {
        if (cars >= N) break;
        uint32_t w0, w1, w2;
        if (draws) {
          const uint32_t* d = draws + ((size_t)e * cfg.G + g) * 3;
          w0 = d[0]; w1 = d[1]; w2 = d[2];
        } else {
          const uint4 w = ic3_draw24(cfg.seed, cfg.env_id0 + (uint32_t)e, tick, IC3_STREAM_TJ_SPAWN, (uint32_t)g);
          w0 = w.x; w1 = w.y; w2 = w.z;
        }
        if (w0 <= cfg.spawn_thr) {
          const unsigned dead = __ballot_sync(IC3_FULL_MASK, lane < N && !alive);
          const int k = __popc(dead);
          const int j = (int)ic3_pick(w1, (uint32_t)k);
          const int slot = (int)__fns(dead, 0, j + 1);
          const int p = (int)ic3_pick(w2, (uint32_t)cfg.P);
          if (lane == slot) {
            alive = 1;
            rid = p + g * cfg.P;
            rpos = 0;
            const int cell = cfg.route_cells[(size_t)rid * cfg.Lmax];
            rr = cell >> 16;
            cc = cell & 0xffff;
          }
          cars += 1;
        }
      }
      int crash = 0;
      for (int j = 0; j < N; ++j) {
        const int rj = __shfl_sync(IC3_FULL_MASK, rr, j), cj = __shfl_sync(IC3_FULL_MASK, cc, j);
        crash |= (j != lane && rj == rr && cj == cc && (rr | cc) != 0);
      }
      crash = (lane < N) ? crash : 0;
      const bool any_crash = __any_sync(IC3_FULL_MASK, crash);
      double rew = -0.01 * (double)wait;
      if (crash) rew += -10.0;
      rew = alive ? rew : 0.0;
      int failed = a.st.has_failed[e];
      failed |= any_crash ? 1 : 0;
      if (lane < N) {
        a.st.loc[i * 2] = rr;
        a.st.loc[i * 2 + 1] = cc;
        a.st.alive[i] = (uint8_t)alive;
        a.st.wait[i] = wait;
        a.st.route_id[i] = rid;
        a.st.route_pos[i] = rpos;
        a.st.last_act[i] = (uint8_t)lact;
        a.st.completed[i] = (uint8_t)completed;
        reward[i] = (float)rew;
      }
      if (lane == 0) {
        a.st.cars_in_sys[e] = cars;
        a.st.has_failed[e] = (uint8_t)failed;
        a.st.tick[e] = tick + 1;
      }
      if (r.has) {
        const bool done_t = ic3_rollout_tail(r.io, e, cfg.B, N, lane, (float)rew, false, (uint8_t)alive,
                                             (uint8_t)completed, 1 - failed);
        if (done_t) {
          __syncwarp();
          tj_reset_env(a, e, lane);
          rr = cc = alive = wait = lact = 0;
          rid = rpos = -1;
        }
      }
    }
    if (do_step && r.has && r.io.snap_T > 0) {
      __syncwarp();
      ic3_rollout_snapshot(r.io, e, cfg.B, N, lane);
      if (r.io.t + 1 < r.io.snap_T && lane < N) {
        const size_t k = ((size_t)(r.io.t + 1) * cfg.B + e) * N + lane;
        if (r.io.snap_tj_loc) {
          r.io.snap_tj_loc[2 * k] = rr;
          r.io.snap_tj_loc[2 * k + 1] = cc;
        }
        if (r.io.snap_tj_alive) r.io.snap_tj_alive[k] = (uint8_t)alive;
        if (r.io.snap_tj_last_act) r.io.snap_tj_last_act[k] = (uint8_t)lact;
        if (r.io.snap_tj_route_id) r.io.snap_tj_route_id[k] = rid;
      }
    }
    if (obs && lane < N) {
      s_r[lane] = rr;
      s_c[lane] = cc;
      s_alive[lane] = alive;
      s_rid[lane] = rid;
      s_lact[lane] = lact;
    }
  }
  if (obs == nullptr) return;
  __syncthreads();
  const int W = 2 * cfg.vision + 1;
  tj_write_obs(cfg, s_r, s_c, s_alive, s_rid, s_lact, s_cell, obs + (size_t)e * N * (2 + W * W * cfg.vocab), keep_l2 != 0);
}

template <int H>
__global__ void __launch_bounds__(128) tj_obs_encode_kernel(TJArgs a, float* __restrict__ obs,
                                                            const float* __restrict__ wT, const float* __restrict__ bias,
                                                            float* __restrict__ x, bool split, int keep_l2) {
  ic3_pdl_trigger();
  ic3_pdl_wait();
  extern __shared__ uint32_t s_cell[];
  __shared__ int s_r[IC3_MAX_AGENTS], s_c[IC3_MAX_AGENTS], s_alive[IC3_MAX_AGENTS], s_rid[IC3_MAX_AGENTS],
      s_lact[IC3_MAX_AGENTS];
  const ic3_tj_cfg& cfg = a.cfg;
  const int N = cfg.N, W = 2 * cfg.vision + 1, WW = W * W, V = cfg.vocab;
  const int e = blockIdx.x, warp = threadIdx.x >> 5, lane = threadIdx.x & 31;
  if (threadIdx.x < N) {
    const size_t i = (size_t)e * N + threadIdx.x;
    s_r[threadIdx.x] = a.st.loc[i * 2];
    s_c[threadIdx.x] = a.st.loc[i * 2 + 1];
    s_alive[threadIdx.x] = a.st.alive[i];
    s_rid[threadIdx.x] = a.st.route_id[i];
    s_lact[threadIdx.x] = a.st.last_act[i];
  }
  __syncthreads();
  tj_write_obs(cfg, s_r, s_c, s_alive, s_rid, s_lact, s_cell, obs + (size_t)e * N * (2 + WW * V), keep_l2 != 0);
  for (int i = warp; i < N; i += blockDim.x >> 5) {
    const uint32_t* rec = s_cell + i * WW;
    const bool alive = s_alive[i] != 0;
    const float la = alive ? (float)s_lact[i] : 0.f;
    const float ri = alive ? (float)s_rid[i] / (float)(cfg.npath - 1) : 0.f;
    tj_encode_row<H>(alive, la, ri, [rec](int w) { return rec[w]; }, WW, V, cfg.car_cls, wT, bias, split,
                     x + ((size_t)e * N + i) * H, lane);
  }
}

__global__ void __launch_bounds__(IC3_OBS_WRITER_THREADS, IC3_OBS_WRITER_MIN_CTAS)
    tj_obs_writer_kernel(TJArgs a, float* __restrict__ obs, int keep_l2) {
  ic3_pdl_trigger();
  ic3_pdl_wait();
  extern __shared__ uint32_t s_cell[];
  __shared__ int s_r[IC3_MAX_AGENTS], s_c[IC3_MAX_AGENTS], s_alive[IC3_MAX_AGENTS], s_rid[IC3_MAX_AGENTS],
      s_lact[IC3_MAX_AGENTS];
  const ic3_tj_cfg& cfg = a.cfg;
  const int N = cfg.N, W = 2 * cfg.vision + 1, B = cfg.B;
  const size_t per_env = (size_t)N * (2 + W * W * cfg.vocab);
  const int k = threadIdx.x;
  int r = 0, c = 0, alive = 0, rid = 0, lact = 0;
  auto load = [&](int e) {
    const size_t i = (size_t)e * N + k;
    r = a.st.loc[i * 2];
    c = a.st.loc[i * 2 + 1];
    alive = a.st.alive[i];
    rid = a.st.route_id[i];
    lact = a.st.last_act[i];
  };
  if (k < N && (int)blockIdx.x < B) load(blockIdx.x);
  for (int e = blockIdx.x; e < B; e += gridDim.x) {
    if (k < N) {
      s_r[k] = r;
      s_c[k] = c;
      s_alive[k] = alive;
      s_rid[k] = rid;
      s_lact[k] = lact;
      if (e + (int)gridDim.x < B) load(e + gridDim.x);
    }
    __syncthreads();
    tj_write_obs(cfg, s_r, s_c, s_alive, s_rid, s_lact, s_cell, obs + (size_t)e * per_env, keep_l2 != 0);
    __syncthreads();
  }
}

int tj_check(const ic3_tj_cfg* cfg, const ic3_tj_state* st) {
  if (!cfg || !st) return IC3_E_NULL;
  if (!st->loc || !st->alive || !st->wait || !st->route_id || !st->route_pos || !st->last_act ||
      !st->completed || !st->cars_in_sys || !st->has_failed || !st->tick)
    return IC3_E_NULL;
  if (!cfg->grid || !cfg->route_len || !cfg->route_cells) return IC3_E_NULL;
  if (cfg->B <= 0 || cfg->N <= 0 || cfg->N > IC3_MAX_AGENTS) return IC3_E_RANGE;
  if (cfg->h <= 0 || cfg->w <= 0 || cfg->h > 32767 || cfg->w > 32767) return IC3_E_RANGE;
  if (cfg->vision < 0 || cfg->vision > 7) return IC3_E_RANGE;
  if (cfg->G <= 0 || cfg->P <= 0 || cfg->Lmax <= 0 || cfg->npath < 2 || cfg->vocab <= 0 || cfg->vocab > 65535)
    return IC3_E_RANGE;
  return IC3_OK;
}

int tj_launch(const ic3_tj_cfg* cfg, const ic3_tj_state* st, const int32_t* act, int act_stride,
              const uint32_t* draws, float* reward, float* obs, int32_t* err, const ic3_rollout_io* r,
              int do_step, cudaStream_t s) {
  TJArgs a{*cfg, *st};
  const int W = 2 * cfg->vision + 1;
  const size_t smem = obs ? (size_t)cfg->N * W * W * sizeof(uint32_t) : 0;
  const int threads = obs ? 128 : 32 * IC3_ENV_WARPS;
  const int grid = obs ? cfg->B : (cfg->B + IC3_ENV_WARPS - 1) / IC3_ENV_WARPS;
  RolloutOpt ro = make_rollout_opt(r);
  const int keep = obs && (size_t)cfg->B * cfg->N * (2 + W * W * cfg->vocab) * sizeof(float) <= IC3_OBS_L2_KEEP_BYTES;
  IC3_LAUNCH_RC(ic3_launch_pdl(tj_step_kernel, dim3(grid), dim3(threads), smem, s, a, act, act_stride, draws, reward, obs, err,
                               ro, do_step, keep));
  return IC3_OK;
}

template <int H>
int tj_obs_encode_launch(const ic3_tj_cfg* cfg, const ic3_tj_state* st, const ic3_policy_cfg* pcfg,
                         const ic3_policy_packed* w, float* obs, float* x, cudaStream_t s) {
  TJArgs a{*cfg, *st};
  const int W = 2 * cfg->vision + 1;
  const size_t smem = (size_t)cfg->N * W * W * sizeof(uint32_t);
  const bool split = pcfg->obs_vocab > 0;
  const int keep = (size_t)cfg->B * cfg->N * (2 + W * W * cfg->vocab) * sizeof(float) <= IC3_OBS_L2_KEEP_BYTES;
  IC3_LAUNCH_RC(ic3_launch_pdl(tj_obs_encode_kernel<H>, dim3(cfg->B), dim3(128), smem, s, a, obs, (const float*)w->enc_wT,
                               (const float*)w->enc_b, x, split, keep));
  return IC3_OK;
}

}

extern "C" int ic3_tj_obs_bounded(const ic3_tj_cfg* cfg, const ic3_tj_state* st, float* obs, void* stream) {
  int rc = tj_check(cfg, st);
  if (rc) return rc;
  if (!obs) return IC3_E_NULL;
  TJArgs a{*cfg, *st};
  const int W = 2 * cfg->vision + 1;
  const size_t smem = (size_t)cfg->N * W * W * sizeof(uint32_t);
  const int keep = (size_t)cfg->B * cfg->N * (2 + W * W * cfg->vocab) * sizeof(float) <= IC3_OBS_L2_KEEP_BYTES;
  int grid = 0;
  rc = ic3_grid_beside_lstm((const void*)tj_obs_writer_kernel, IC3_OBS_WRITER_THREADS, smem, cfg->B, &grid);
  if (rc) return rc;
  IC3_LAUNCH_RC(ic3_launch_pdl(tj_obs_writer_kernel, dim3(grid), dim3(IC3_OBS_WRITER_THREADS), smem,
                               (cudaStream_t)stream, a, obs, keep));
  return IC3_OK;
}

extern "C" int ic3_tj_reset(const ic3_tj_cfg* cfg, const ic3_tj_state* st, const uint8_t* mask,
                            float* obs, void* stream) {
  int rc = tj_check(cfg, st);
  if (rc) return rc;
  cudaStream_t s = (cudaStream_t)stream;
  TJArgs a{*cfg, *st};
  const int wpb = 4;
  tj_reset_kernel<<<(cfg->B + wpb - 1) / wpb, wpb * 32, 0, s>>>(a, mask);
  IC3_LAUNCH_CHECK();
  if (obs) return tj_launch(cfg, st, nullptr, 0, nullptr, nullptr, obs, nullptr, nullptr, 0, s);
  return IC3_OK;
}

extern "C" int ic3_tj_step(const ic3_tj_cfg* cfg, const ic3_tj_state* st, const int32_t* act,
                           int32_t act_stride, const uint32_t* draws, float* reward, float* obs,
                           int32_t* err, const ic3_rollout_io* r, void* stream) {
  int rc = tj_check(cfg, st);
  if (rc) return rc;
  if (!act || !reward || !err || act_stride < 1) return IC3_E_NULL;
  if (r && (!r->t_ep || !r->fresh || !r->alive_next || (r->hard_attn && (!r->comm_next || !r->action))))
    return IC3_E_NULL;
  return tj_launch(cfg, st, act, act_stride, draws, reward, obs, err, r, 1, (cudaStream_t)stream);
}

extern "C" int ic3_tj_obs(const ic3_tj_cfg* cfg, const ic3_tj_state* st, float* obs, void* stream) {
  int rc = tj_check(cfg, st);
  if (rc) return rc;
  if (!obs) return IC3_E_NULL;
  return tj_launch(cfg, st, nullptr, 0, nullptr, nullptr, obs, nullptr, nullptr, 0, (cudaStream_t)stream);
}

extern "C" int ic3_tj_obs_encode(const ic3_tj_cfg* env, const ic3_tj_state* st, const ic3_policy_cfg* cfg,
                                 const ic3_policy_packed* w, float* obs, float* x, void* stream) {
  int rc = tj_check(env, st);
  if (rc) return rc;
  rc = ic3_encoder_check(cfg, w);
  if (rc) return rc;
  if (!obs || !x) return IC3_E_NULL;
  if (env->B != cfg->B || env->N != cfg->N) return IC3_E_RANGE;
  const int W = 2 * env->vision + 1;
  if (cfg->O != 2 + W * W * env->vocab) return IC3_E_RANGE;
  rc = ic3_tj_layout_check(env, cfg);
  if (rc) return rc;
  IC3_DISPATCH_H(cfg->H, tj_obs_encode_launch<HH>(env, st, cfg, w, obs, x, (cudaStream_t)stream));
}
```

ic3net_b200/trainer.py:

```python
import ctypes as C
import math
from collections import namedtuple

import torch
import torch.nn.functional as F

from . import _lib
from .optim import FlatRMSprop
from .utils import merge_stat

Transition = namedtuple('Transition', ('state', 'action', 'action_out', 'value', 'episode_mask',
                                       'episode_mini_mask', 'next_state', 'reward', 'misc'))

RolloutBatch = namedtuple('RolloutBatch', ('action', 'logp', 'value', 'reward', 'episode_mask',
                                           'episode_mini_mask', 'alive_mask', 'valid'))


def policy_forward_torch(net, x, h, c, g, n_alive):
    w, cp = net._kernel_weights(), net._cfg_proto
    B, N = g.shape
    H = x.shape[1]
    lstm = cp['cell'] == _lib.CELL_LSTM
    if cp['x_tanh']:
        x = torch.tanh(x)
    hid = x if cp['h_from_x'] else h
    den = torch.where(n_alive > 1, n_alive - 1, torch.ones_like(n_alive)) if cp['comm_avg'] else torch.ones_like(n_alive)
    gg = g.unsqueeze(-1)
    for ps in range(max(1, cp['passes'])):
        if cp['comm_mask_zero'] or N < 2:
            S = torch.zeros_like(hid)
        else:
            hv = hid.view(B, N, H)
            tot = (gg * hv).sum(1, keepdim=True)
            S = (gg * (tot - gg * hv) / den.unsqueeze(-1)).reshape(B * N, H)
        cvec = F.linear(S, w['c_w'][ps], w['c_b'][ps])
        if lstm:
            gates = F.linear(x + cvec, w['w_ih'], w['b_ih']) + F.linear(hid, w['w_hh'], w['b_hh'])
            gi, gf, gq, go = gates.chunk(4, dim=1)
            c = torch.sigmoid(gf) * c + torch.sigmoid(gi) * torch.tanh(gq)
            hid = torch.sigmoid(go) * torch.tanh(c)
        else:
            hid = torch.tanh(x + F.linear(hid, w['f_w'][ps], w['f_b'][ps]) + cvec)
    value = F.linear(hid, w['value_w'], w['value_b'])
    logps = [F.log_softmax(F.linear(hid, hw, hb), dim=-1) for hw, hb in zip(w['head_w'], w['head_b'])]
    return hid, c, value, logps


class Trainer(object):
    def __init__(self, args, policy_net, env):
        if not hasattr(policy_net, 'packed'):
            raise NotImplementedError("Trainer drives policies that run on the CUDA kernels (CommNetMLP, models.MLP, "
                                      "models.RNN); models.Random has no kernel path")
        self.args = args
        self.policy_net = policy_net
        self.env = env
        self.display = False
        self.last_step = False
        self.optimizer = FlatRMSprop(policy_net.parameters(), lr=args.lrate, alpha=0.97, eps=1e-6)
        self.params = [p for p in self.policy_net.parameters()]
        self.obs_mode = getattr(args, 'obs_mode', 'index')
        self.use_graph = bool(getattr(args, 'use_graph', False))
        self.is_tj = args.env_name == 'traffic_junction'
        self.record_for_grad = bool(getattr(args, 'record_for_grad', False))
        self.grad_window = int(getattr(args, 'grad_window', 40))
        self.grad_impl = getattr(args, 'grad_impl', None) or 'auto'
        self.grad_kernels = False
        self._bptt = None
        self._buf = None
        self._graph = None
        self._graph_key = None
        self._side = None
        policy_net.set_obs_layout(*getattr(env.env, 'obs_layout', (0, 0, 0)))
        self.use_xtable = bool(getattr(args, 'encoder_table', True))
        self._xtable = None
        self._xtable_key = None
        if self.record_for_grad and self.grad_impl in ('auto', 'kernels'):
            ok = self._bptt_supported()
            if self.grad_impl == 'kernels' and not ok:
                raise NotImplementedError("grad_impl='kernels' needs the tensor-core policy path (hid_size 128), the "
                                          "per-position encoder table, <= 7 action logits and a small vision window")
            self.grad_kernels = ok
        if self.grad_impl == 'auto':
            self.grad_impl = 'kernels' if self.grad_kernels else 'autograd'

    def _bptt_supported(self):
        e, net = self.env.env, self.policy_net
        W = 2 * e.vision + 1
        if net.policy_impl != 'tc' or not self.use_xtable or W * W > 25 or 1 + sum(self.args.naction_heads) > 8:
            return False
        if getattr(net, 'is_variant', False):
            return False
        if getattr(e, 'obs_layout', (0, 0, 0))[1] == 0:
            return False
        npos = e.obs_positions
        used = npos + ((W * W + 4) if self.is_tj else (2 * W * W + 1))
        return (used + 15) // 16 * 16 <= 512

    def _encoder_table(self, cfg, w):
        e, net = self.env.env, self.policy_net
        if not self.use_xtable or cfg.obs_vocab == 0:
            return None
        key = net._packed_key
        if self._xtable is None:
            self._xtable = torch.empty(e.obs_positions, net.hid_size, device=e.device)
        if key != self._xtable_key:
            fn = _lib.load().ic3_tj_encoder_table if self.is_tj else _lib.load().ic3_pp_encoder_table
            _lib.check(fn(C.byref(e.cfg), C.byref(cfg), C.byref(w), self._xtable.data_ptr(), _lib.stream()))
            self._xtable_key = key
        return self._xtable

    def _alloc(self, T):
        e = self.env.env
        B, N, H = e.nenvs, self.args.nagents, self.args.hid_size
        dev = e.device
        nh = len(self.args.naction_heads)
        A = sum(self.args.naction_heads)
        z = lambda *s, dtype=torch.float32: torch.zeros(*s, dtype=dtype, device=dev)
        b = dict(T=T, h=z(B * N, H), c=z(B * N, H), x=z(B * N, H),
                 comm=z(B, N, dtype=torch.uint8), alive=torch.ones(B, N, dtype=torch.uint8, device=dev),
                 fresh=torch.ones(B, dtype=torch.uint8, device=dev), t_ep=z(B, dtype=torch.int32),
                 action=z(T, B, N, nh, dtype=torch.int32), logp=z(T, B, N, A), value=z(T, B * N),
                 reward=z(T, B, N), emask=z(T, B, dtype=torch.uint8), mini=z(T, B, N, dtype=torch.uint8),
                 ralive=z(T, B, N, dtype=torch.uint8), step_reward=z(B, N),
                 stat_reward=z(B, N), stat_comm=z(B, N), stat_success=z(B, dtype=torch.int32),
                 stat_episodes=z(B, dtype=torch.int32), stat_steps=z(B, dtype=torch.int32),
                 err=z(1, dtype=torch.int32), halted=z(B, dtype=torch.uint8), valid=z(T, B, dtype=torch.uint8),
                 statvec=z(4 + 2 * N, dtype=torch.float64))
        if self.obs_mode == 'dense' or (self.record_for_grad and self.is_tj and not self.grad_kernels):
            b['obs'] = torch.empty(B, N, self.env.observation_dim, dtype=torch.float32, device=dev)
        if self.record_for_grad and self.grad_kernels:
            b.update(s_fresh=z(T, B, dtype=torch.uint8), s_comm=z(T, B, N, dtype=torch.uint8),
                     s_alive=z(T, B, N, dtype=torch.uint8), s_tep=z(T, B, dtype=torch.int32),
                     rec_h=torch.empty(T + 1, B * N, H, device=dev), rec_c=torch.empty(T + 1, B * N, H, device=dev))
            if self.is_tj:
                b.update(s_tjloc=z(T, B, N, 2, dtype=torch.int32), s_tjalive=z(T, B, N, dtype=torch.uint8),
                         s_tjlast=z(T, B, N, dtype=torch.uint8), s_tjroute=z(T, B, N, dtype=torch.int32))
            else:
                b['s_loc'] = z(T, B, e.npredator + 1, 2, dtype=torch.int32)
        elif self.record_for_grad:
            W = self.grad_window
            nw = (T + W - 1) // W
            b.update(s_fresh=z(T, B, dtype=torch.uint8), s_comm=z(T, B, N, dtype=torch.uint8),
                     s_alive=z(T, B, N, dtype=torch.uint8), s_tep=z(T, B, dtype=torch.int32),
                     ck_h=z(nw, B * N, H), ck_c=z(nw, B * N, H))
            if self.is_tj:
                b['s_obs'] = z(T, B, N, self.env.observation_dim)
            else:
                b['s_loc'] = z(T, B, e.npredator + 1, 2, dtype=torch.int32)
        self._buf = b
        self._graph = None
        return b

    def _dense_chunks(self, cfg):
        e, b = self.env.env, self._buf
        B, N, O, H = e.nenvs, self.args.nagents, self.env.observation_dim, self.args.hid_size
        key = (B, b['obs'].data_ptr(), b['x'].data_ptr(), cfg.obs_vocab, cfg.seed, cfg.env_id0)
        if getattr(self, '_chunks_key', None) == key:
            return self._chunks
        mb = float(getattr(self.args, 'obs_chunk_mb', 0) or 0)
        per_env = N * O * 4
        nchunk = max(1, -(-B * per_env // int(mb * (1 << 20)))) if mb > 0 else 1
        step = -(-B // nchunk)
        out = []
        for k0 in range(0, B, step):
            k1 = min(B, k0 + step)
            ecfg, est = e.chunk_view(k0, k1)
            ccfg = _lib.PolicyCfg.from_buffer_copy(cfg)
            ccfg.B, ccfg.env_id0 = k1 - k0, cfg.env_id0 + k0
            out.append((ecfg, est, ccfg, b['obs'].data_ptr() + k0 * per_env, b['x'].data_ptr() + k0 * N * H * 4))
        self._chunks, self._chunks_key = out, key
        return out

    def _fused_x(self):
        dense = self.obs_mode == 'dense' or (self.record_for_grad and self.is_tj and not self.grad_kernels)
        W = 2 * self.env.env.vision + 1
        return (not dense) and self.policy_net.policy_impl == 'tc' and W * W <= 25

    OVERLAP_MIN_OBS_BYTES = 8 << 20

    def _overlap_obs(self):
        if self.obs_mode != 'dense' or (self.record_for_grad and self.is_tj and not self.grad_kernels):
            return False
        e = self.env.env
        if e.nenvs * self.args.nagents * self.env.observation_dim * 4 < self.OVERLAP_MIN_OBS_BYTES:
            return False
        W = 2 * e.vision + 1
        return self.policy_net.policy_impl == 'tc' and W * W <= 25

    def _enqueue(self, T, quota=0):
        b, e, net, args = self._buf, self.env.env, self.policy_net, self.args
        lib = _lib.load()
        B, N = e.nenvs, args.nagents
        nh = len(args.naction_heads)
        cfg = net.policy_cfg(B)
        cfg.seed, cfg.env_id0 = e.cfg.seed, e.cfg.env_id0
        w = net.packed()
        hard = int(bool(args.hard_attn) and bool(args.commnet))
        s = _lib.stream()
        ws, _ = net.workspace(B)
        rec = self.record_for_grad
        gk = rec and self.grad_kernels
        dense = self.obs_mode == 'dense' or (rec and self.is_tj and not gk)
        overlap = self._overlap_obs()
        fused_x = self._fused_x() or overlap
        src = {}
        if fused_x:
            src = dict(tj_env=C.addressof(e.cfg), tj_state=C.addressof(e.state)) if self.is_tj else \
                dict(pp_env=C.addressof(e.cfg), pp_state=C.addressof(e.state))
            src['x_table'] = None if overlap else _lib.ptr(self._encoder_table(cfg, w))
        if overlap:
            main = torch.cuda.current_stream()
            if self._side is None or self._side.device != main.device:
                self._side = torch.cuda.Stream(device=main.device)
            side = self._side
            obs_write = lib.ic3_tj_obs_bounded if self.is_tj else lib.ic3_pp_obs_bounded
        fuse_heads = (net.policy_impl == 'tc' and 1 + sum(args.naction_heads) <= 8 and ws is not None
                      and bool(getattr(args, 'fuse_heads', False)))
        heads_kw = {}
        if fuse_heads:
            hd = (C.c_int32 * _lib.MAX_HEADS)(*(list(args.naction_heads) + [0] * (_lib.MAX_HEADS - nh)))
            heads_kw = dict(head_partial=lib.ic3_policy_partial_ptr(C.byref(cfg), ws.data_ptr()),
                            head_b=net._bufs['head_b'].data_ptr(), head_dim=hd)
        snap = {}
        if rec:
            snap = dict(snap_T=T, snap_fresh=b['s_fresh'].data_ptr(), snap_comm=b['s_comm'].data_ptr(),
                        snap_alive=b['s_alive'].data_ptr(), snap_tep=b['s_tep'].data_ptr())
            if not self.is_tj:
                snap['snap_pp_loc'] = b['s_loc'].data_ptr()
            elif gk:
                snap.update(snap_tj_loc=b['s_tjloc'].data_ptr(), snap_tj_alive=b['s_tjalive'].data_ptr(),
                            snap_tj_last_act=b['s_tjlast'].data_ptr(), snap_tj_route_id=b['s_tjroute'].data_ptr())
        for t in range(T):
            if rec:
                if t == 0:
                    b['s_fresh'][0].copy_(b['fresh'])
                    b['s_comm'][0].copy_(b['comm'])
                    b['s_alive'][0].copy_(b['alive'])
                    b['s_tep'][0].copy_(b['t_ep'])
                    if not self.is_tj:
                        b['s_loc'][0].copy_(e.loc)
                    elif gk:
                        b['s_tjloc'][0].copy_(e.car_loc)
                        b['s_tjalive'][0].copy_(e.alive_mask)
                        b['s_tjlast'][0].copy_(e.car_last_act)
                        b['s_tjroute'][0].copy_(e.route_id)
                if not gk and t % self.grad_window == 0:
                    b['ck_h'][t // self.grad_window].copy_(b['h'])
                    b['ck_c'][t // self.grad_window].copy_(b['c'])
            if overlap:
                side.wait_stream(main)
                for ecfg, est, _, o_ptr, _ in self._dense_chunks(cfg):
                    _lib.check(obs_write(C.byref(ecfg), C.byref(est), o_ptr, side.cuda_stream))
            elif dense:
                obs_enc = lib.ic3_tj_obs_encode if self.is_tj else lib.ic3_pp_obs_encode
                for ecfg, est, ccfg, o_ptr, x_ptr in self._dense_chunks(cfg):
                    _lib.check(obs_enc(C.byref(ecfg), C.byref(est), C.byref(ccfg), C.byref(w), o_ptr, x_ptr, s))
                if rec and self.is_tj:
                    b['s_obs'][t].copy_(b['obs'])
            elif fused_x:
                pass
            elif self.is_tj:
                _lib.check(lib.ic3_tj_encoder_index(C.byref(e.cfg), C.byref(e.state), C.byref(cfg), C.byref(w),
                                                    b['x'].data_ptr(), s))
            else:
                _lib.check(lib.ic3_pp_encoder_index(C.byref(e.cfg), C.byref(e.state), C.byref(cfg), C.byref(w),
                                                    b['x'].data_ptr(), s))
            hin, cin = (b['rec_h'][t], b['rec_c'][t]) if gk else (b['h'], b['c'])
            hout, cout = (b['rec_h'][t + 1], b['rec_c'][t + 1]) if gk else (b['h'], b['c'])
            io = _lib.PolicyIO(x=None if fused_x else b['x'].data_ptr(), h=hin.data_ptr(), c=cin.data_ptr(),
                               comm_action=b['comm'].data_ptr() if hard else None, alive=b['alive'].data_ptr(),
                               fresh=b['fresh'].data_ptr(), tick=e.tick.data_ptr(), draws=None,
                               h_out=hout.data_ptr(), c_out=cout.data_ptr(), value=b['value'][t].data_ptr(),
                               logp=b['logp'][t].data_ptr(), action=b['action'][t].data_ptr(),
                               workspace=_lib.ptr(ws), err=b['err'].data_ptr(), defer_heads=int(fuse_heads), **src)
            _lib.check(lib.ic3_policy_step(C.byref(cfg), C.byref(w), C.byref(io), s))
            if fuse_heads:
                heads_kw.update(head_value=b['value'][t].data_ptr(), head_logp=b['logp'][t].data_ptr())
            if overlap:
                main.wait_stream(side)
            r = _lib.RolloutIO(t=t, max_steps=args.max_steps, nheads=nh, hard_attn=hard,
                               comm_action_one=int(bool(args.comm_action_one)),
                               last=int(t == T - 1 and quota <= 0), batch_size=int(quota),
                               halted=b['halted'].data_ptr(), rec_valid=b['valid'].data_ptr(), **snap, **heads_kw,
                               action=b['action'][t].data_ptr(), t_ep=b['t_ep'].data_ptr(),
                               fresh=b['fresh'].data_ptr(), comm_next=b['comm'].data_ptr(),
                               alive_next=b['alive'].data_ptr(), rec_reward=b['reward'].data_ptr(),
                               rec_episode_mask=b['emask'].data_ptr(), rec_mini_mask=b['mini'].data_ptr(),
                               rec_alive=b['ralive'].data_ptr(), stat_reward=b['stat_reward'].data_ptr(),
                               stat_comm=b['stat_comm'].data_ptr(), stat_success=b['stat_success'].data_ptr(),
                               stat_episodes=b['stat_episodes'].data_ptr(), stat_steps=b['stat_steps'].data_ptr())
            if self.is_tj:
                _lib.check(lib.ic3_tj_step(C.byref(e.cfg), C.byref(e.state), b['action'][t].data_ptr(), nh, None,
                                           b['step_reward'].data_ptr(), None, b['err'].data_ptr(), C.byref(r), s))
            else:
                _lib.check(lib.ic3_pp_step(C.byref(e.cfg), C.byref(e.state), b['action'][t].data_ptr(), nh,
                                           b['step_reward'].data_ptr(), None, b['err'].data_ptr(), C.byref(r), s))

    def _episode_boundary(self, epoch):
        e, b = self.env.env, self._buf
        if self.is_tj:
            e.reset(epoch, want_obs=False)
        else:
            e.reset(want_obs=False)
        for k in ('stat_reward', 'stat_comm', 'stat_success', 'stat_episodes', 'stat_steps', 't_ep', 'halted'):
            b[k].zero_()
        b['fresh'].fill_(1)

    def rollout(self, T, epoch=0, quota=0):
        e = self.env.env
        if self._buf is None or self._buf['T'] != T:
            self._alloc(T)
        b = self._buf
        self._episode_boundary(epoch)
        b['err'].zero_()
        w = self.policy_net.packed()
        if self._fused_x():
            self._encoder_table(self.policy_net.policy_cfg(e.nenvs), w)
        if self.use_graph:
            key = (T, int(quota), int(getattr(e.cfg, 'spawn_thr', 0)), int(e.cfg.seed), int(e.cfg.env_id0))
            if self._graph is None or self._graph_key != key:
                snap = e.snapshot()
                keys = ('fresh', 'comm', 'alive', 't_ep', 'h', 'c', 'halted', 'stat_reward', 'stat_comm', 'stat_success',
                        'stat_episodes', 'stat_steps')
                saved = {k: b[k].clone() for k in keys}
                self._enqueue(T, quota)
                torch.cuda.synchronize()
                e.restore(snap)
                for k, v in saved.items():
                    b[k].copy_(v)
                g = torch.cuda.CUDAGraph()
                with torch.cuda.graph(g):
                    self._enqueue(T, quota)
                self._graph, self._graph_key = g, key
                g.replay()
            else:
                self._graph.replay()
        else:
            self._enqueue(T, quota)
        return RolloutBatch(action=b['action'], logp=b['logp'], value=b['value'].view(T, e.nenvs, -1),
                            reward=b['reward'], episode_mask=b['emask'], episode_mini_mask=b['mini'],
                            alive_mask=b['ralive'], valid=b['valid'])

    def stat_vector(self):
        b, e = self._buf, self.env.env
        hard = bool(self.args.hard_attn) and bool(self.args.commnet)
        _lib.check(_lib.load().ic3_stat_reduce(e.nenvs, self.args.nagents, b['stat_episodes'].data_ptr(),
                                               b['stat_steps'].data_ptr(), b['stat_success'].data_ptr(),
                                               b['err'].data_ptr(), b['stat_reward'].data_ptr(),
                                               b['stat_comm'].data_ptr() if hard else None,
                                               b['statvec'].data_ptr(), _lib.stream()))
        return b['statvec']

    def stat_from_vector(self, v):
        args, N = self.args, self.args.nagents
        flags = int(v[3])
        if flags:
            raise RuntimeError("device-side error flag %#x during rollout" % flags)
        stat = dict()
        stat['num_episodes'] = int(round(float(v[0])))
        stat['num_steps'] = int(round(float(v[1])))
        stat['steps_taken'] = stat['num_steps']
        nf = int(getattr(args, 'nfriendly', N))
        enemy = bool(getattr(args, 'enemy_comm', False))
        stat['reward'] = v[4:4 + nf].copy()
        if enemy:
            stat['enemy_reward'] = v[4 + nf:4 + N].copy()
        if args.hard_attn and args.commnet:
            stat['comm_action'] = v[4 + N:4 + N + nf].copy()
            if enemy:
                stat['enemy_comm'] = v[4 + N + nf:4 + 2 * N].copy()
        if not (not self.is_tj and args.mode == 'competitive'):
            stat['success'] = int(round(float(v[2])))
        if self.is_tj:
            stat['add_rate'] = self.env.env.add_rate * stat['num_episodes']
        return stat

    def collect_stat(self):
        return self.stat_from_vector(self.stat_vector().cpu().numpy())

    def get_episode(self, epoch):
        batch = self.rollout(self.args.max_steps, epoch, quota=1)
        return batch, self.collect_stat()

    def episodes_end_early(self):
        return (not self.is_tj) and getattr(self.args, 'mode', 'mixed') == 'mixed'

    def batch_plan(self):
        bs, ms = int(self.args.batch_size), int(self.args.max_steps)
        full = int(math.ceil(bs / float(ms))) * ms
        if getattr(self.args, 'batch_boundary', 'reference') == 'cut':
            return full, 0
        return (bs + ms - 1 if self.episodes_end_early() else full), bs

    def steps_per_batch(self):
        return self.batch_plan()[0]

    def run_batch(self, epoch):
        T, quota = self.batch_plan()
        batch = self.rollout(T, epoch, quota=quota)
        self.stats = self.collect_stat()
        return batch, self.stats

    def _pp_sparse_obs(self, loc):
        e = self.env.env
        D, v, N = e.dim, e.vision, e.npredator
        NA = e.nagent_rows
        W, V = 2 * v + 1, e.vocab_size
        loc = loc.long()
        pr, pc = loc[:, :N, 0], loc[:, :N, 1]
        ar = torch.arange(W, device=loc.device)
        dy, dx = ar.repeat_interleave(W), ar.repeat(W)
        rr = loc[:, :NA, 0].unsqueeze(-1) - v + dy
        cc = loc[:, :NA, 1].unsqueeze(-1) - v + dx
        inside = (rr >= 0) & (rr < D) & (cc >= 0) & (cc < D)
        base = torch.arange(W * W, device=loc.device) * V
        cls = torch.where(inside, rr * D + cc, torch.full_like(rr, D * D + 1)) + base
        npred = ((rr.unsqueeze(-1) == pr[:, None, None, :]) & (cc.unsqueeze(-1) == pc[:, None, None, :])).sum(-1)
        nprey = (rr == loc[:, N:, 0].unsqueeze(-1)) & (cc == loc[:, N:, 1].unsqueeze(-1))
        idx = torch.cat([cls, (base + V - 2).expand_as(cls), (base + V - 1).expand_as(cls)], -1)
        val = torch.cat([torch.ones_like(cls), nprey.long() * inside, npred * inside], -1).float()
        return idx.reshape(-1, 3 * W * W), val.reshape(-1, 3 * W * W)

    def _forward_window(self, t0, t1, h, c, adv, ret):
        b, net, args = self._buf, self.policy_net, self.args
        B, N, H = self.env.env.nenvs, args.nagents, args.hid_size
        hard = bool(args.hard_attn) and bool(args.commnet)
        w = net._kernel_weights()
        w_e, b_e = w['enc_w'], w['enc_b']
        w_eT = None if self.is_tj else w_e.t().contiguous()
        loss = torch.zeros((), device=h.device)
        st = dict(action_loss=torch.zeros((), device=h.device), value_loss=torch.zeros((), device=h.device),
                  entropy=torch.zeros((), device=h.device))
        for t in range(t0, t1):
            keep = (1 - b['s_fresh'][t].float()).repeat_interleave(N).unsqueeze(1)
            h, c = h * keep, c * keep
            if self.is_tj:
                x = F.linear(b['s_obs'][t].reshape(B * N, -1), w_e, b_e)
            else:
                idx, val = self._pp_sparse_obs(b['s_loc'][t])
                x = F.embedding_bag(idx, w_eT, per_sample_weights=val, mode='sum') + b_e
            fresh = b['s_fresh'][t].bool().unsqueeze(1)
            alive = torch.where(fresh, torch.ones_like(b['s_alive'][t]), b['s_alive'][t]).float()
            n_alive = alive.sum(1, keepdim=True)
            g = alive
            if hard:
                g = g * torch.where(fresh, torch.zeros_like(b['s_comm'][t]), b['s_comm'][t]).float()
            h, c, value, logps = policy_forward_torch(net, x, h, c, g, n_alive)
            value = value.view(B, N)
            alive_post = b['ralive'][t].float()
            act = b['action'][t].long()
            lp_taken = torch.zeros(B, N, device=h.device)
            ent = torch.zeros((), device=h.device)
            vmask = b['valid'][t].float().view(B, 1, 1)
            for k, lp in enumerate(logps):
                lp = lp.view(B, N, -1)
                lp_taken = lp_taken + lp.gather(-1, act[..., k:k + 1]).squeeze(-1)
                ent = ent - (lp * lp.exp() * vmask).sum()
            a_loss = (-adv[t] * lp_taken * alive_post).sum()
            v_loss = ((value - ret[t]).pow(2) * alive_post).sum()
            step_loss = a_loss + args.value_coeff * v_loss
            if args.entr > 0:
                step_loss = step_loss - args.entr * ent
            loss = loss + step_loss
            st['action_loss'] += a_loss.detach(); st['value_loss'] += v_loss.detach(); st['entropy'] += ent.detach()
            det = (((b['s_tep'][t] + 1) % args.detach_gap) == 0).repeat_interleave(N).unsqueeze(1)
            if bool(args.detach_gap <= self.args.max_steps):
                h = torch.where(det, h.detach(), h)
                c = torch.where(det, c.detach(), c)
        return loss, h, c, st

    LOSS_KEYS = ('action_loss', 'value_loss', 'entropy')

    def compute_grad(self, batch):
        v = self.compute_grad_device(batch).cpu().numpy()
        return {k: float(v[i]) for i, k in enumerate(self.LOSS_KEYS)}

    def compute_grad_device(self, batch):
        if not self.record_for_grad:
            raise RuntimeError("set args.record_for_grad = True before the rollout to use compute_grad")
        b, args = self._buf, self.args
        e = self.env.env
        T, B, N = b['T'], e.nenvs, args.nagents
        ret = torch.empty(T, B, N, device=e.device)
        _lib.check(_lib.load().ic3_returns_scan(T, B, N, float(args.gamma), float(args.mean_ratio),
                                                b['reward'].data_ptr(), b['emask'].data_ptr(), b['mini'].data_ptr(),
                                                ret.data_ptr(), _lib.stream()))
        adv = ret - b['value'].view(T, B, N)
        if args.normalize_rewards:
            v = b['valid'].float().unsqueeze(-1)
            cnt = v.sum(0, keepdim=True) * N
            mean = (adv * v).sum((0, 2), keepdim=True) / cnt
            var = (((adv - mean) * v) ** 2).sum((0, 2), keepdim=True) / (cnt - 1)
            adv = (adv - mean) / var.sqrt()
        if self.grad_kernels:
            return self._compute_grad_kernels(adv, ret)
        W = self.grad_window
        nw = (T + W - 1) // W
        dh = dc = None
        if self.grad_impl == 'manual':
            tot = self._compute_grad_manual(adv, ret, W, nw)
            return torch.tensor([tot[k] for k in self.LOSS_KEYS], dtype=torch.float64, device=e.device)
        tot = torch.zeros(3, dtype=torch.float64, device=e.device)
        for k in reversed(range(nw)):
            t0, t1 = k * W, min(T, (k + 1) * W)
            h0 = b['ck_h'][k].clone().requires_grad_(True)
            c0 = b['ck_c'][k].clone().requires_grad_(True)
            loss, h1, c1, st = self._forward_window(t0, t1, h0, c0, adv, ret)
            if dh is not None:
                loss = loss + (h1 * dh).sum() + (c1 * dc).sum()
            loss.backward()
            dh = h0.grad.detach() if h0.grad is not None else torch.zeros_like(h0)
            dc = c0.grad.detach() if c0.grad is not None else torch.zeros_like(c0)
            tot += torch.stack([st[key] for key in self.LOSS_KEYS]).double()
        return tot

    def _compute_grad_kernels(self, adv, ret):
        b, net, args, e = self._buf, self.policy_net, self.args, self.env.env
        lib = _lib.load()
        T, B, N, H = b['T'], e.nenvs, args.nagents, args.hid_size
        s = _lib.stream()
        cfg = net.policy_cfg(B)
        cfg.seed, cfg.env_id0 = e.cfg.seed, e.cfg.env_id0
        w = net.packed()
        table = self._encoder_table(cfg, w)
        if self._bptt is None or self._bptt['B'] != B:
            plan = _lib.BpttPlan(cfg=C.pointer(cfg), w=C.pointer(w),
                                 pp_env=None if self.is_tj else C.pointer(e.cfg),
                                 tj_env=C.pointer(e.cfg) if self.is_tj else None, x_table=table.data_ptr(),
                                 value_coeff=float(args.value_coeff), entr=float(args.entr), workspace=None)
            nbytes = int(lib.ic3_bptt_workspace_bytes(C.byref(plan)))
            if nbytes == 0:
                raise NotImplementedError("this configuration is outside the BPTT kernels (use grad_impl='autograd')")
            self._bptt = dict(B=B, ws=torch.empty(nbytes, dtype=torch.uint8, device=e.device),
                              dh=torch.zeros(B * N, H, device=e.device), dc=torch.zeros(B * N, H, device=e.device),
                              losses=torch.zeros(3, dtype=torch.float64, device=e.device))
        st = self._bptt
        plan = _lib.BpttPlan(cfg=C.pointer(cfg), w=C.pointer(w), pp_env=None if self.is_tj else C.pointer(e.cfg),
                             tj_env=C.pointer(e.cfg) if self.is_tj else None, x_table=table.data_ptr(),
                             value_coeff=float(args.value_coeff), entr=float(args.entr), workspace=st['ws'].data_ptr())
        hard = bool(args.hard_attn) and bool(args.commnet)
        adv = adv.contiguous()
        cut = None
        if args.detach_gap <= args.max_steps:
            cut = (((b['s_tep'] + 1) % args.detach_gap) == 0).to(torch.uint8).contiguous()
        lo, hi = torch.aminmax(b['rec_c'][1:])
        cmax = max(abs(float(lo.item())), abs(float(hi.item())))
        st['dh'].zero_()
        st['dc'].zero_()
        _lib.check(lib.ic3_bptt_begin(C.byref(plan), cmax, s))
        value = b['value']

        def step_io(t):
            return _lib.BpttStepIO(t=t, h_prev=b['rec_h'][t].data_ptr(), c_prev=b['rec_c'][t].data_ptr(),
                                   h_new=b['rec_h'][t + 1].data_ptr(), fresh=b['s_fresh'][t].data_ptr(),
                                   comm=b['s_comm'][t].data_ptr() if hard else None, alive=b['s_alive'][t].data_ptr(),
                                   cut=cut[t].data_ptr() if cut is not None else None,
                                   pp_loc=None if self.is_tj else b['s_loc'][t].data_ptr(),
                                   tj_loc=b['s_tjloc'][t].data_ptr() if self.is_tj else None,
                                   tj_alive=b['s_tjalive'][t].data_ptr() if self.is_tj else None,
                                   tj_last_act=b['s_tjlast'][t].data_ptr() if self.is_tj else None,
                                   tj_route_id=b['s_tjroute'][t].data_ptr() if self.is_tj else None,
                                   logp=b['logp'][t].data_ptr(), action=b['action'][t].data_ptr(),
                                   value=value[t].data_ptr(), ret=ret[t].data_ptr(), adv=adv[t].data_ptr(),
                                   alive_post=b['ralive'][t].data_ptr(), valid=b['valid'][t].data_ptr(),
                                   dh=st['dh'].data_ptr(), dc=st['dc'].data_ptr(), err=b['err'].data_ptr())
        nxt = step_io(T - 1) if T > 0 else None
        if nxt is not None:
            _lib.check(lib.ic3_bptt_prepare(C.byref(plan), C.byref(nxt), s))
        for t in reversed(range(T)):
            io = nxt
            if t > 0:
                nxt = step_io(t - 1)
                _lib.check(lib.ic3_bptt_prepare(C.byref(plan), C.byref(nxt), s))
            _lib.check(lib.ic3_bptt_step(C.byref(plan), C.byref(io), s))
        params, grads = self._param_structs()
        _lib.check(lib.ic3_bptt_finish(C.byref(plan), C.byref(params), C.byref(grads), st['losses'].data_ptr(), s))
        return st['losses']

    def _param_structs(self):
        net = self.policy_net
        w = net._kernel_weights()
        scratch = self.__dict__.setdefault('_grad_scratch', {})

        def grad_ptr(p):
            if isinstance(p, torch.nn.Parameter):
                if p.grad is None:
                    p.grad = torch.zeros_like(p)
                return p.grad.data_ptr()
            key = p.data_ptr()
            if key not in scratch:
                scratch[key] = torch.zeros_like(p)
            return scratch[key].data_ptr()

        def mk(get):
            arr = lambda lst: (C.c_void_p * _lib.MAX_HEADS)(*([get(t) for t in lst] + [None] * (_lib.MAX_HEADS - len(lst))))
            return _lib.PolicyParams(encoder_w=get(w['enc_w']), encoder_b=get(w['enc_b']), c_w=get(w['c_w'][0]),
                                     c_b=get(w['c_b'][0]), w_ih=get(w['w_ih']), w_hh=get(w['w_hh']), b_ih=get(w['b_ih']),
                                     b_hh=get(w['b_hh']), value_w=get(w['value_w']), value_b=get(w['value_b']),
                                     head_w=arr(w['head_w']), head_b=arr(w['head_b']))
        return mk(lambda p: p.data_ptr()), mk(grad_ptr)

    def _compute_grad_manual(self, adv, ret, W, nw):
        from . import bptt
        b, net, args = self._buf, self.policy_net, self.args
        if getattr(net, 'is_variant', False) or type(net).__name__ != 'CommNetMLP':
            raise NotImplementedError("grad_impl='manual' covers the recurrent LSTM CommNet / IC3Net with one comm pass")
        B, N = self.env.env.nenvs, args.nagents
        T = b['T']
        P, G = {}, {}
        for name, p in net.named_parameters():
            if p.grad is None:
                p.grad = torch.zeros_like(p)
            P[name], G[name] = p.detach(), p.grad
        spec = bptt.Spec(N, args.hid_size, len(args.naction_heads), bool(args.hard_attn) and bool(args.commnet),
                         getattr(args, 'comm_mode', 'avg') == 'avg', bool(args.comm_mask_zero), args.value_coeff,
                         args.entr, args.detach_gap, args.max_steps)
        if self.is_tj:
            obs_fn = lambda t: b['s_obs'][t].reshape(B * N, -1)
        else:
            obs_fn = lambda t: self._pp_sparse_obs(b['s_loc'][t])
        rec = dict(fresh=b['s_fresh'], comm=b['s_comm'], alive=b['s_alive'], t_ep=b['s_tep'], action=b['action'],
                   alive_post=b['ralive'], obs=obs_fn, valid=b['valid'])
        tot = dict(action_loss=0.0, value_loss=0.0, entropy=0.0)
        dh = dc = None
        for k in reversed(range(nw)):
            t0, t1 = k * W, min(T, (k + 1) * W)
            dh, dc, st = bptt.window_backward(P, G, spec, rec, t0, t1, b['ck_h'][k], b['ck_c'][k], adv, ret, dh, dc)
            for key in tot:
                tot[key] += st[key]
        return tot

    def train_batch(self, epoch):
        batch, stat = self.run_batch(epoch)
        self.optimizer.zero_grad(set_to_none=False)
        s = self.compute_grad(batch)
        merge_stat(s, stat)
        self.optimizer.step(grad_div=stat['num_steps'])
        return stat

    def state_dict(self):
        return self.optimizer.state_dict()

    def load_state_dict(self, state):
        self.optimizer.load_state_dict(state)
```

include/ic3net_b200.h:

```cpp
#ifndef IC3NET_B200_H
#define IC3NET_B200_H

#include <stdint.h>

#ifdef __cplusplus
extern "C" {
#endif

#define IC3_MAX_AGENTS 32
#define IC3_MAX_HEADS 4
#define IC3_MAX_HEAD_DIM 16

enum {
  IC3_OK = 0,
  IC3_E_NULL = -1,
  IC3_E_RANGE = -2,
  IC3_E_UNSUPPORTED = -3
};

enum {
  IC3_ERR_EPISODE_DONE = 1,
  IC3_ERR_ROUTE_OVERRUN = 2,
  IC3_ERR_BAD_ACTION = 4,
  IC3_ERR_PIPELINE = 0x100,
  IC3_ERR_FP16_RANGE = 0x200
};

enum { IC3_PP_MIXED = 0, IC3_PP_COOPERATIVE = 1, IC3_PP_COMPETITIVE = 2 };

const char* ic3_version(void);
const char* ic3_strerror(int code);
uint64_t ic3_launch_count(void);

typedef struct {
  int32_t B;
  int32_t N;
  int32_t dim;
  int32_t vision;
  int32_t mode;
  int32_t naction;
  uint32_t env_id0;
  int32_t enemy_comm;
  uint64_t seed;
} ic3_pp_cfg;

typedef struct {
  int32_t* loc;
  uint8_t* reached;
  uint8_t* done;
  int32_t* success;
  uint32_t* episode;
  uint32_t* tick;
} ic3_pp_state;

typedef struct {
  int32_t t;
  int32_t max_steps;
  int32_t nheads;
  int32_t hard_attn;
  int32_t comm_action_one;
  int32_t last;
  const int32_t* action;
  int32_t* t_ep;
  uint8_t* fresh;
  uint8_t* comm_next;
  uint8_t* alive_next;
  float* rec_reward;
  uint8_t* rec_episode_mask;
  uint8_t* rec_mini_mask;
  uint8_t* rec_alive;
  float* stat_reward;
  float* stat_comm;
  int32_t* stat_success;
  int32_t* stat_episodes;
  int32_t* stat_steps;
  int32_t batch_size;
  int32_t reserved0;
  uint8_t* halted;
  uint8_t* rec_valid;
  int32_t snap_T;
  int32_t reserved1;
  uint8_t* snap_fresh;
  uint8_t* snap_comm;
  uint8_t* snap_alive;
  int32_t* snap_tep;
  int32_t* snap_pp_loc;
  int32_t* snap_tj_loc;
  uint8_t* snap_tj_alive;
  uint8_t* snap_tj_last_act;
  int32_t* snap_tj_route_id;
  const float* head_partial;
  const float* head_b;
  float* head_value;
  float* head_logp;
  int32_t head_dim[IC3_MAX_HEADS];
} ic3_rollout_io;

int ic3_pp_reset(const ic3_pp_cfg* cfg, const ic3_pp_state* st, const uint8_t* mask,
                 float* obs, void* stream);
int ic3_pp_step(const ic3_pp_cfg* cfg, const ic3_pp_state* st, const int32_t* act, int32_t act_stride,
                float* reward, float* obs, int32_t* err, const ic3_rollout_io* r, void* stream);
int ic3_pp_obs(const ic3_pp_cfg* cfg, const ic3_pp_state* st, float* obs, void* stream);
int ic3_pp_obs_bounded(const ic3_pp_cfg* cfg, const ic3_pp_state* st, float* obs, void* stream);

typedef struct {
  int32_t B, N, vision;
  int32_t h, w;
  int32_t G, P, Lmax;
  int32_t outside_cls;
  int32_t car_cls;
  int32_t vocab;
  int32_t npath;
  uint32_t spawn_thr;
  uint32_t env_id0;
  uint64_t seed;
  const int32_t* grid;
  const int32_t* route_len;
  const int32_t* route_cells;
} ic3_tj_cfg;

typedef struct {
  int32_t* loc;
  uint8_t* alive;
  int32_t* wait;
  int32_t* route_id;
  int32_t* route_pos;
  uint8_t* last_act;
  uint8_t* completed;
  int32_t* cars_in_sys;
  uint8_t* has_failed;
  uint32_t* tick;
} ic3_tj_state;

int ic3_tj_reset(const ic3_tj_cfg* cfg, const ic3_tj_state* st, const uint8_t* mask,
                 float* obs, void* stream);
int ic3_tj_step(const ic3_tj_cfg* cfg, const ic3_tj_state* st, const int32_t* act, int32_t act_stride,
                const uint32_t* draws, float* reward, float* obs, int32_t* err,
                const ic3_rollout_io* r, void* stream);
int ic3_tj_obs(const ic3_tj_cfg* cfg, const ic3_tj_state* st, float* obs, void* stream);
int ic3_tj_obs_bounded(const ic3_tj_cfg* cfg, const ic3_tj_state* st, float* obs, void* stream);

typedef struct {
  int32_t B, N, H, O;
  int32_t nheads;
  int32_t head_dim[IC3_MAX_HEADS];
  int32_t hard_attn;
  int32_t comm_avg;
  int32_t comm_mask_zero;
  uint32_t env_id0;
  uint64_t seed;
  int32_t obs_off, obs_vocab, obs_ncount;
  int32_t cell, passes, x_tanh, h_from_x;
  int32_t reserved0;
} ic3_policy_cfg;

enum { IC3_CELL_LSTM = 0, IC3_CELL_TANH = 1 };
#define IC3_MAX_PASSES 4

typedef struct {
  const float* encoder_w;
  const float* encoder_b;
  const float* c_w;
  const float* c_b;
  const float* w_ih;
  const float* w_hh;
  const float* b_ih;
  const float* b_hh;
  const float* value_w;
  const float* value_b;
  const float* head_w[IC3_MAX_HEADS];
  const float* head_b[IC3_MAX_HEADS];
  const float* c_w_pass[IC3_MAX_PASSES];
  const float* c_b_pass[IC3_MAX_PASSES];
  const float* f_w_pass[IC3_MAX_PASSES];
  const float* f_b_pass[IC3_MAX_PASSES];
} ic3_policy_params;

typedef struct {
  float* enc_wT;
  float* enc_b;
  float* c_wT;
  float* c_b;
  float* lstm_wT;
  float* lstm_b;
  float* head_w;
  float* head_b;
  void* lstm_img;
  float* bias_cat;
  float* f_wT;
  float* f_b;
  int32_t* flags;
} ic3_policy_packed;

#define IC3_LSTM_IMG_BYTES 786432

int ic3_policy_pack(const ic3_policy_cfg* cfg, const ic3_policy_params* p,
                    const ic3_policy_packed* out, void* stream);

int ic3_encoder_dense(const ic3_policy_cfg* cfg, const ic3_policy_packed* w, const float* obs,
                      float* x, void* stream);
int ic3_pp_encoder_index(const ic3_pp_cfg* env, const ic3_pp_state* st, const ic3_policy_cfg* cfg,
                         const ic3_policy_packed* w, float* x, void* stream);
int ic3_tj_encoder_index(const ic3_tj_cfg* env, const ic3_tj_state* st, const ic3_policy_cfg* cfg,
                         const ic3_policy_packed* w, float* x, void* stream);
int ic3_pp_obs_encode(const ic3_pp_cfg* env, const ic3_pp_state* st, const ic3_policy_cfg* cfg,
                      const ic3_policy_packed* w, float* obs, float* x, void* stream);
int ic3_tj_obs_encode(const ic3_tj_cfg* env, const ic3_tj_state* st, const ic3_policy_cfg* cfg,
                      const ic3_policy_packed* w, float* obs, float* x, void* stream);
int ic3_pp_encoder_table(const ic3_pp_cfg* env, const ic3_policy_cfg* cfg, const ic3_policy_packed* w,
                         float* table, void* stream);
int ic3_tj_encoder_table(const ic3_tj_cfg* env, const ic3_policy_cfg* cfg, const ic3_policy_packed* w,
                         float* table, void* stream);

typedef struct {
  const float* x;
  const float* h;
  const float* c;
  const uint8_t* comm_action;
  const uint8_t* alive;
  const uint8_t* fresh;
  const uint32_t* tick;
  const uint32_t* draws;
  float* h_out;
  float* c_out;
  float* value;
  float* logp;
  int32_t* action;
  void* workspace;
  int32_t* err;
  const ic3_pp_cfg* pp_env;
  const ic3_pp_state* pp_state;
  const ic3_tj_cfg* tj_env;
  const ic3_tj_state* tj_state;
  const float* x_table;
  int32_t defer_heads;
  int32_t pass_index;
} ic3_policy_io;

const float* ic3_policy_partial_ptr(const ic3_policy_cfg* cfg, const void* workspace);

uint64_t ic3_policy_workspace_bytes(const ic3_policy_cfg* cfg);

int ic3_policy_step(const ic3_policy_cfg* cfg, const ic3_policy_packed* w, const ic3_policy_io* io,
                    void* stream);
int ic3_policy_step_profile(const ic3_policy_cfg* cfg, const ic3_policy_packed* w, const ic3_policy_io* io,
                            void* stream, float* ms);
int ic3_sample_actions(const ic3_policy_cfg* cfg, const float* logp, const uint32_t* tick,
                       const uint32_t* draws, int32_t* action, void* stream);

int ic3_returns_scan(int32_t T, int32_t B, int32_t N, float gamma, float mean_ratio, const float* reward,
                     const uint8_t* episode_mask, const uint8_t* mini_mask, float* returns, void* stream);

int ic3_stat_reduce(int32_t B, int32_t N, const int32_t* stat_episodes, const int32_t* stat_steps,
                    const int32_t* stat_success, const int32_t* err, const float* stat_reward,
                    const float* stat_comm, double* out, void* stream);

typedef struct {
  const ic3_policy_cfg* cfg;
  const ic3_policy_packed* w;
  const ic3_pp_cfg* pp_env;
  const ic3_tj_cfg* tj_env;
  const float* x_table;
  float value_coeff;
  float entr;
  void* workspace;
} ic3_bptt_plan;

typedef struct {
  int32_t t;
  int32_t reserved0;
  const float* h_prev;
  const float* c_prev;
  const float* h_new;
  const uint8_t* fresh;
  const uint8_t* comm;
  const uint8_t* alive;
  const uint8_t* cut;
  const int32_t* pp_loc;
  const int32_t* tj_loc;
  const uint8_t* tj_alive;
  const uint8_t* tj_last_act;
  const int32_t* tj_route_id;
  const float* logp;
  const int32_t* action;
  const float* value;
  const float* ret;
  const float* adv;
  const uint8_t* alive_post;
  const uint8_t* valid;
  float* dh;
  float* dc;
  int32_t* err;
} ic3_bptt_step_io;

uint64_t ic3_bptt_workspace_bytes(const ic3_bptt_plan* plan);
int ic3_bptt_begin(const ic3_bptt_plan* plan, float c_abs_max, void* stream);
int ic3_bptt_step(const ic3_bptt_plan* plan, const ic3_bptt_step_io* io, void* stream);
int ic3_bptt_prepare(const ic3_bptt_plan* plan, const ic3_bptt_step_io* io, void* stream);
int ic3_bptt_finish(const ic3_bptt_plan* plan, const ic3_policy_params* params, const ic3_policy_params* grads,
                    double* losses, void* stream);

int ic3_rmsprop_step(int64_t n, float lr, float alpha, float eps, float grad_div, float* grad,
                     float* param, float* square_avg, void* stream);

#ifdef __cplusplus
}
#endif
#endif
```

Measured before the change: 100.7 million.

## Fuse dense observation writes into prep and LSTM kernels, drop side stream

Dense observation rows are no longer written by a separate obs-writer kernel on a side stream. The prep kernel now writes most rows directly. For large observation buffers it leaves a tail of rows as compact class records, and extra writer warps in the LSTM tensor-core kernel expand those records into observations using bulk shared-to-global copies while the MMA warps run. This removes a kernel launch, the side-stream waits and a second read of the environment state. In exchange the LSTM kernel carries extra warps and shared memory, and a small record buffer is added to the workspace.

```diff
diff --git a/ic3net_b200/_lib.py b/ic3net_b200/_lib.py
--- a/ic3net_b200/_lib.py
+++ b/ic3net_b200/_lib.py
@@ -83,7 +83,8 @@
     _fields_ = [("x", _p), ("h", _p), ("c", _p), ("comm_action", _p), ("alive", _p), ("fresh", _p), ("tick", _p),
                 ("draws", _p), ("h_out", _p), ("c_out", _p), ("value", _p), ("logp", _p), ("action", _p),
                 ("workspace", _p), ("err", _p), ("pp_env", _p), ("pp_state", _p), ("tj_env", _p), ("tj_state", _p),
-                ("x_table", _p), ("defer_heads", C.c_int32), ("pass_index", C.c_int32)]
+                ("x_table", _p), ("defer_heads", C.c_int32), ("pass_index", C.c_int32), ("obs", _p),
+                ("obs_lstm_rows", C.c_int32)]
 
 
 class BpttPlan(C.Structure):
diff --git a/ic3net_b200/csrc/obs_rows.cuh b/ic3net_b200/csrc/obs_rows.cuh
--- /dev/null
+++ b/ic3net_b200/csrc/obs_rows.cuh
@@ -0,0 +1,47 @@
+#pragma once
+#include "ic3_common.cuh"
+
+namespace {
+
+template <bool VEC4>
+__device__ __forceinline__ void pp_store_cell(uint32_t info, float* __restrict__ dst, int V, int lane, bool keep) {
+  const int cls = (int)(info & 0xffffu);
+  const float npred = (float)((info >> 16) & 0xffu), nprey = (float)(info >> 24);
+  if (VEC4) {
+    const int V4 = V >> 2, qc = cls >> 2, qp = (V - 1) >> 2, qy = (V - 2) >> 2;
+    for (int q = lane; q < V4; q += 32) {
+      float4 o = make_float4(0.f, 0.f, 0.f, 0.f);
+      if (q == qc) {
+        const int k = cls & 3;
+        o.x = k == 0 ? 1.f : 0.f; o.y = k == 1 ? 1.f : 0.f; o.z = k == 2 ? 1.f : 0.f; o.w = k == 3 ? 1.f : 0.f;
+      }
+      if (q == qy) {
+        o.z = nprey;
+      }
+      if (q == qp) {
+        o.w = npred;
+      }
+      ic3_st_obs(reinterpret_cast<float4*>(dst) + q, o, keep);
+    }
+  } else {
+    for (int q = lane; q < V; q += 32) {
+      float o = (q == cls) ? 1.f : 0.f;
+      if (q == V - 2) o = nprey;
+      if (q == V - 1) o = npred;
+      ic3_st_obs(dst + q, o, keep);
+    }
+  }
+}
+
+__device__ __forceinline__ void tj_store_cell(uint32_t info, bool live, int car_cls, float* __restrict__ dst, int V,
+                                              int lane, bool keep) {
+  const int cls = (int)(info & 0xffffu);
+  const float cnt = (float)(info >> 16);
+  for (int q = lane; q < V; q += 32) {
+    float o = (q == cls) ? 1.f : 0.f;
+    if (q == car_cls) o += cnt;
+    ic3_st_obs(dst + q, live ? o : 0.f, keep);
+  }
+}
+
+}
diff --git a/ic3net_b200/csrc/policy_tc.cu b/ic3net_b200/csrc/policy_tc.cu
--- a/ic3net_b200/csrc/policy_tc.cu
+++ b/ic3net_b200/csrc/policy_tc.cu
@@ -4,11 +4,10 @@
 
 
 constexpr int TC_TILE_PAD = 8;
-constexpr size_t LSTM_SMEM_BYTES = NSTAGE_P * STAGE_BYTES + 256 + TC_H * HEAD_PAD * sizeof(float) + 4 * TC_H * sizeof(float);
 
 static int ctas_beside_lstm(const void* kern, int threads, size_t smem, int* per_sm, int* nsm) {
   cudaFuncAttributes la, ka;
-  cudaError_t e = cudaFuncGetAttributes(&la, lstm_tc_kernel);
+  cudaError_t e = cudaFuncGetAttributes(&la, lstm_tc_kernel<0>);
   if (e == cudaSuccess) e = cudaFuncGetAttributes(&ka, kern);
   int dev = 0, regs = 0, smem_sm = 0, reserved = 0, thr_sm = 0, blk_sm = 0;
   if (e == cudaSuccess) e = cudaGetDevice(&dev);
@@ -50,15 +49,19 @@
   return IC3_OK;
 }
 
+template <int OW>
 static int launch_lstm(const ic3_policy_cfg* cfg, const ic3_policy_io* io, const ic3_policy_packed* w, const __half* a_img,
-                       int ntiles_pad, size_t smem, int nout, float* partial, cudaStream_t s) {
+                       int ntiles_pad, size_t smem, int nout, float* partial, const ObsRows& ob, cudaStream_t s) {
   static int max_ctas = 0;
-  auto kern = lstm_tc_kernel;
-  if (max_ctas == 0) {
+  static size_t smem_set = 0;
+  auto kern = lstm_tc_kernel<OW>;
+  constexpr int threads = TC_P_THREADS + 32 * OW;
+  if (max_ctas == 0 || smem > smem_set) {
     cudaError_t e = cudaFuncSetAttribute(kern, cudaFuncAttributeMaxDynamicSharedMemorySize, (int)smem);
+    smem_set = smem;
     if (e != cudaSuccess) return (int)e;
     int per_sm = 0, dev = 0, nsm = 0;
-    e = cudaOccupancyMaxActiveBlocksPerMultiprocessor(&per_sm, kern, TC_P_THREADS, smem);
+    e = cudaOccupancyMaxActiveBlocksPerMultiprocessor(&per_sm, kern, threads, smem);
     if (e == cudaSuccess) e = cudaGetDevice(&dev);
     if (e == cudaSuccess) e = cudaDeviceGetAttribute(&nsm, cudaDevAttrMultiProcessorCount, dev);
     if (e != cudaSuccess || per_sm <= 0) return e != cudaSuccess ? (int)e : IC3_E_RANGE;
@@ -67,7 +70,7 @@
   const int nitems = 2 * ntiles_pad;
   cudaLaunchConfig_t lc{};
   lc.gridDim = dim3(nitems < max_ctas ? nitems : max_ctas);
-  lc.blockDim = dim3(TC_P_THREADS);
+  lc.blockDim = dim3(threads);
   lc.dynamicSmemBytes = smem;
   lc.stream = s;
   cudaLaunchAttribute la[1];
@@ -77,7 +80,7 @@
   const __half* b_img = reinterpret_cast<const __half*>(w->lstm_img) + (size_t)io->pass_index * B_IMG_HALFS;
   cudaError_t e = cudaLaunchKernelEx(&lc, kern, *cfg, *io, a_img, b_img,
                                      (const float*)w->bias_cat + (size_t)io->pass_index * 4 * TC_H, nitems,
-                                     (const float*)w->head_w, nout, partial);
+                                     (const float*)w->head_w, nout, partial, ob);
   ++g_ic3_launches;
   return e == cudaSuccess ? IC3_OK : (int)e;
 }
@@ -88,7 +91,8 @@
   const long ntiles = (R + TC_M - 1) / TC_M;
   const long ntiles_pad = (ntiles + TC_TILE_PAD - 1) / TC_TILE_PAD * TC_TILE_PAD;
   const uint64_t carry = cfg->passes > 1 ? (uint64_t)4 * R * TC_H * sizeof(float) : 0;
-  return (uint64_t)ntiles_pad * TC_NCHUNK * A_CHUNK_BYTES + (uint64_t)R * NSLOT * HEAD_PAD * sizeof(float) + carry;
+  return (uint64_t)ntiles_pad * TC_NCHUNK * A_CHUNK_BYTES + (uint64_t)R * NSLOT * HEAD_PAD * sizeof(float) +
+         (uint64_t)R * OBS_REC_W * sizeof(uint32_t) + carry;
 }
 
 extern "C" const float* ic3_policy_partial_ptr(const ic3_policy_cfg* cfg, const void* workspace) {
@@ -153,6 +157,19 @@
 }
 
 static int tc_pass(const ic3_policy_cfg* cfg, const ic3_policy_packed* w, const ic3_policy_io* io, cudaStream_t s, bool last);
+
+template <int XSRC, bool OBS>
+static cudaError_t launch_prep(const ic3_policy_cfg* cfg, const ic3_policy_io* io, __half* img, const PrepSrc& src,
+                               int ntiles_pad, cudaStream_t s) {
+  static bool cfgd = false;
+  if (!cfgd) {
+    cudaError_t e = cudaFuncSetAttribute(prep_kernel<XSRC, false, false, OBS>, cudaFuncAttributeMaxDynamicSharedMemorySize, PREP_X_BYTES + (PREP_ROWS + 2) * TC_H * 4);
+    if (e != cudaSuccess) return e;
+    cfgd = true;
+  }
+  return ic3_launch_pdl(prep_kernel<XSRC, false, false, OBS>, dim3(2 * ntiles_pad), dim3(256), PREP_X_BYTES + prep_T_bytes(cfg->N), s, *cfg, *io, img, src, PrepBwd{});
+}
+
 
 int ic3_tc_policy_step(const ic3_policy_cfg* cfg, const ic3_policy_packed* w, const ic3_policy_io* io, cudaStream_t s) {
   if (cfg->H != TC_H) return IC3_E_UNSUPPORTED;
@@ -194,6 +211,28 @@
   src.table = io->x_table;
   src.wflags = w->flags;
   if (src.table && !src.split) return IC3_E_RANGE;
+  const bool obs = io->obs && io->pass_index == 0;
+  if (io->obs) {
+    if (io->x || src.table || !(io->pp_env || io->tj_env)) return IC3_E_RANGE;
+    if (io->obs_lstm_rows < 0 || io->obs_lstm_rows > PREP_ROWS) return IC3_E_RANGE;
+  }
+  if (obs) {
+    src.ob.obs = io->obs;
+    src.ob.rec = reinterpret_cast<uint32_t*>(reinterpret_cast<unsigned char*>(io->workspace) +
+                                             (size_t)ntiles_pad * TC_NCHUNK * A_CHUNK_BYTES +
+                                             (size_t)R * NSLOT * HEAD_PAD * sizeof(float));
+    src.ob.rows = io->obs_lstm_rows;
+    src.ob.O = cfg->O;
+    src.ob.keep = (size_t)R * cfg->O * sizeof(float) <= IC3_OBS_L2_KEEP_BYTES;
+    src.ob.pace = 1;
+    int dev = 0, optin = 0;
+    cudaError_t e = cudaGetDevice(&dev);
+    if (e == cudaSuccess) e = cudaDeviceGetAttribute(&optin, cudaDevAttrMaxSharedMemoryPerBlockOptin, dev);
+    if (e != cudaSuccess) return (int)e;
+    if (cfg->O % 4 != 0 || (reinterpret_cast<uintptr_t>(io->obs) & 15) != 0 ||
+        LSTM_SMEM_BYTES + 2 * (size_t)cfg->O * sizeof(float) > (size_t)optin)
+      src.ob.rows = 0;
+  }
   prof_mark(0, s);
   if (io->x) {
     IC3_LAUNCH_RC(ic3_launch_pdl(prep_kernel<XSRC_TENSOR, false>, dim3(2 * ntiles_pad), dim3(PREP_THREADS), prep_T_bytes(cfg->N), s, *cfg, *io, img, src, PrepBwd{}));
@@ -206,14 +245,13 @@
     if (int lrc = ic3_pp_layout_check(io->pp_env, cfg)) return lrc;
     if (src.table) {
       IC3_LAUNCH_RC(ic3_launch_pdl(prep_kernel<XSRC_PP, true>, dim3(2 * ntiles_pad), dim3(PREP_THREADS), prep_T_bytes(cfg->N), s, *cfg, *io, img, src, PrepBwd{}));
+    } else if (obs) {
+      const int V = io->pp_env->dim * io->pp_env->dim + 4;
+      src.ob.WW = W * W; src.ob.V = V;
+      src.ob.vec4 = V % 4 == 0 && (reinterpret_cast<uintptr_t>(io->obs) & 15) == 0;
+      IC3_LAUNCH_RC((launch_prep<XSRC_PP, true>(cfg, io, img, src, ntiles_pad, s)));
     } else {
-      static bool cfgd = false;
-      if (!cfgd) {
-        cudaError_t e = cudaFuncSetAttribute(prep_kernel<XSRC_PP, false>, cudaFuncAttributeMaxDynamicSharedMemorySize, PREP_X_BYTES + (PREP_ROWS + 2) * TC_H * 4);
-        if (e != cudaSuccess) return (int)e;
-        cfgd = true;
-      }
-      IC3_LAUNCH_RC(ic3_launch_pdl(prep_kernel<XSRC_PP, false>, dim3(2 * ntiles_pad), dim3(256), PREP_X_BYTES + prep_T_bytes(cfg->N), s, *cfg, *io, img, src, PrepBwd{}));
+      IC3_LAUNCH_RC((launch_prep<XSRC_PP, false>(cfg, io, img, src, ntiles_pad, s)));
     }
   } else if (io->tj_env && io->tj_state) {
     const int W = 2 * io->tj_env->vision + 1;
@@ -224,27 +262,27 @@
     if (int lrc = ic3_tj_layout_check(io->tj_env, cfg)) return lrc;
     if (src.table) {
       IC3_LAUNCH_RC(ic3_launch_pdl(prep_kernel<XSRC_TJ, true>, dim3(2 * ntiles_pad), dim3(PREP_THREADS), prep_T_bytes(cfg->N), s, *cfg, *io, img, src, PrepBwd{}));
+    } else if (obs) {
+      src.ob.WW = W * W; src.ob.V = io->tj_env->vocab;
+      src.ob.tj = 1; src.ob.car_cls = io->tj_env->car_cls;
+      IC3_LAUNCH_RC((launch_prep<XSRC_TJ, true>(cfg, io, img, src, ntiles_pad, s)));
     } else {
-      static bool cfgd = false;
-      if (!cfgd) {
-        cudaError_t e = cudaFuncSetAttribute(prep_kernel<XSRC_TJ, false>, cudaFuncAttributeMaxDynamicSharedMemorySize, PREP_X_BYTES + (PREP_ROWS + 2) * TC_H * 4);
-        if (e != cudaSuccess) return (int)e;
-        cfgd = true;
-      }
-      IC3_LAUNCH_RC(ic3_launch_pdl(prep_kernel<XSRC_TJ, false>, dim3(2 * ntiles_pad), dim3(256), PREP_X_BYTES + prep_T_bytes(cfg->N), s, *cfg, *io, img, src, PrepBwd{}));
+      IC3_LAUNCH_RC((launch_prep<XSRC_TJ, false>(cfg, io, img, src, ntiles_pad, s)));
     }
   } else {
     return IC3_E_NULL;
   }
   prof_mark(1, s);
-  const size_t smem = LSTM_SMEM_BYTES;
+  const size_t smem = obs && src.ob.rows > 0 ? LSTM_SMEM_BYTES + 2 * (size_t)cfg->O * sizeof(float) : LSTM_SMEM_BYTES;
   int nout = 1;
   for (int k = 0; k < cfg->nheads; ++k) nout += cfg->head_dim[k];
   const bool fused_heads = nout <= HEAD_PAD;
   float* partial = fused_heads ? reinterpret_cast<float*>(reinterpret_cast<unsigned char*>(io->workspace) +
                                                            (size_t)ntiles_pad * TC_NCHUNK * A_CHUNK_BYTES)
                                : nullptr;
-  const int rc = launch_lstm(cfg, io, w, img, ntiles_pad, smem, nout, partial, s);
+  const int rc = obs && src.ob.rows > 0
+                     ? launch_lstm<OBS_WARPS>(cfg, io, w, img, ntiles_pad, smem, nout, partial, src.ob, s)
+                     : launch_lstm<0>(cfg, io, w, img, ntiles_pad, smem, nout, partial, ObsRows{}, s);
   if (rc) return rc;
   prof_mark(2, s);
   if (!last) return IC3_OK;
diff --git a/ic3net_b200/csrc/policy_tc_kernels.cuh b/ic3net_b200/csrc/policy_tc_kernels.cuh
--- a/ic3net_b200/csrc/policy_tc_kernels.cuh
+++ b/ic3net_b200/csrc/policy_tc_kernels.cuh
@@ -5,6 +5,7 @@
 #include <cstring>
 
 #include "ic3_common.cuh"
+#include "obs_rows.cuh"
 #include "policy_heads.cuh"
 #include "policy_internal.h"
 #include "tc_common.cuh"
@@ -72,6 +73,28 @@
 constexpr int PREP_X_BYTES = PREP_ROWS * TC_H * 4;
 
 enum { XSRC_TENSOR = 0, XSRC_PP = 1, XSRC_TJ = 2 };
+
+constexpr int OBS_REC_W = PREP_MAX_WW + 3;
+struct ObsRows {
+  float* obs;
+  uint32_t* rec;
+  int rows;
+  int O, WW, V;
+  int tj;
+  int car_cls;
+  int vec4;
+  int keep;
+  int pace;
+};
+
+template <int XSRC>
+__device__ __forceinline__ void obs_store_cell(const ObsRows& ob, size_t row, int w, uint32_t info, bool live, int lane) {
+  float* dst = ob.obs + row * ob.O + (XSRC == XSRC_TJ ? 2 : 0) + (size_t)w * ob.V;
+  if (XSRC == XSRC_TJ) tj_store_cell(info, live, ob.car_cls, dst, ob.V, lane, ob.keep != 0);
+  else if (ob.vec4) pp_store_cell<true>(info, dst, ob.V, lane, ob.keep != 0);
+  else pp_store_cell<false>(info, dst, ob.V, lane, ob.keep != 0);
+}
+
 struct PrepSrc {
   ic3_pp_cfg pp;
   ic3_pp_state pps;
@@ -82,6 +105,7 @@
   const float* table;
   int split;
   const int32_t* wflags;
+  ObsRows ob;
 };
 
 __device__ __forceinline__ void fma4(float4& a, float v, const float4 w) {
@@ -101,11 +125,12 @@
   int npos;
 };
 
-template <int XSRC, bool TAB, bool BWD = false>
+template <int XSRC, bool TAB, bool BWD = false, bool OBS = false>
 __global__ void __launch_bounds__(256) prep_kernel(ic3_policy_cfg cfg, ic3_policy_io io, __half* __restrict__ img,
                                                    PrepSrc src, PrepBwd bw) {
   static_assert(!(TAB && XSRC == XSRC_TENSOR), "the table belongs to the fused index encoder");
   static_assert(!BWD || TAB, "the backward pass uses the per-position table form of the encoder");
+  static_assert(!OBS || (XSRC != XSRC_TENSOR && !TAB), "the observation rows are built from the class records");
   __shared__ float s_gate[PREP_ROWS + 64];
   __shared__ float s_den[PREP_ROWS + 64];
   __shared__ int s_feat[(XSRC == XSRC_TENSOR || TAB) ? 1 : PREP_ROWS * PREP_MAX_WW];
@@ -371,6 +396,41 @@
     store_split4(img, cell + 1 * SEC, cell + 1 * SEC + LO, sv, SCALE_A);
     store_split4(img, cell + 2 * SEC, cell + 2 * SEC + LO, hv, SCALE_A);
   }
+  if constexpr (OBS) {
+    const ObsRows& ob = src.ob;
+    const int WW = ob.WW, V = ob.V, cbase = XSRC == XSRC_TJ ? 2 : 0;
+    auto record = [&](int rl, int w) -> uint32_t {
+      const int cls = s_feat[rl * WW + w] - cbase - w * V, cnt = s_cnt[rl * WW + w];
+      if (XSRC == XSRC_TJ) return (uint32_t)cls | ((uint32_t)cnt << 16);
+      return (uint32_t)cls | ((uint32_t)(cnt & 255) << 16) | ((uint32_t)(cnt >> 8) << 24);
+    };
+    const int nprep = PREP_ROWS - ob.rows;
+    const int nst = min(nprep, R - row0);
+    for (int it = warp; it < nst * WW; it += (blockDim.x >> 5)) {
+      const int rl = it / WW, w = it - rl * WW;
+      obs_store_cell<XSRC>(ob, (size_t)(row0 + rl), w, record(rl, w), XSRC == XSRC_TJ && s_live[rl], lane);
+    }
+    if (XSRC == XSRC_TJ) {
+      for (int rl = threadIdx.x; rl < nst; rl += blockDim.x) {
+        float* dst = ob.obs + (size_t)(row0 + rl) * ob.O;
+        dst[0] = s_live[rl] ? s_la[rl] : 0.f;
+        dst[1] = s_live[rl] ? s_ri[rl] : 0.f;
+      }
+    }
+    const int nrec = min(PREP_ROWS, R - row0) - nprep;
+    for (int p = threadIdx.x; p < nrec * WW; p += blockDim.x) {
+      const int rl = nprep + p / WW, w = p - (rl - nprep) * WW;
+      ob.rec[(size_t)(row0 + rl) * OBS_REC_W + w] = record(rl, w);
+    }
+    if (XSRC == XSRC_TJ) {
+      for (int p = threadIdx.x; p < nrec; p += blockDim.x) {
+        uint32_t* rc = ob.rec + (size_t)(row0 + nprep + p) * OBS_REC_W + PREP_MAX_WW;
+        rc[0] = (uint32_t)s_live[nprep + p];
+        rc[1] = __float_as_uint(s_la[nprep + p]);
+        rc[2] = __float_as_uint(s_ri[nprep + p]);
+      }
+    }
+  }
 }
 
 __device__ __forceinline__ float ex2_fast(float x) {
@@ -425,6 +485,7 @@
 constexpr int MMA_WARPS = 8;
 constexpr int TC_P_THREADS = MMA_WARPS * 32 + 32;
 constexpr int NSLOT = IC3_HEAD_NSLOT;
+constexpr size_t LSTM_SMEM_BYTES = NSTAGE_P * STAGE_BYTES + 256 + TC_H * HEAD_PAD * sizeof(float) + 4 * TC_H * sizeof(float);
 
 template <int NCHUNK>
 __device__ __forceinline__ void wg_gemm_item(float (&d)[128], uint32_t smem_base, uint32_t a_row, uint32_t bar_full,
@@ -562,14 +623,89 @@
   }
 }
 
-__global__ void __launch_bounds__(TC_P_THREADS, 1) lstm_tc_kernel(ic3_policy_cfg cfg, ic3_policy_io io,
+__device__ __forceinline__ void bulk_s2g(float* dst, uint32_t src, uint32_t bytes, bool evict_first) {
+  if (evict_first)
+    asm volatile("{\n\t.reg .b64 pol;\n\tcreatepolicy.fractional.L2::evict_first.b64 pol, 1.0;\n\t"
+                 "cp.async.bulk.global.shared::cta.bulk_group.L2::cache_hint [%0], [%1], %2, pol;\n\t}"
+                 ::"l"(dst), "r"(src), "r"(bytes) : "memory");
+  else
+    asm volatile("cp.async.bulk.global.shared::cta.bulk_group [%0], [%1], %2;" ::"l"(dst), "r"(src), "r"(bytes) : "memory");
+  asm volatile("cp.async.bulk.commit_group;" ::: "memory");
+}
+
+__device__ __forceinline__ void lstm_obs_writer(const ObsRows& ob, float* buf, const volatile int* s_done, int R,
+                                                    int nitems, int lane) {
+  const int WW = ob.WW, V = ob.V, O = ob.O;
+  for (int i = lane; i < 2 * O; i += 32) buf[i] = 0.f;
+  int set0 = -1, set1 = -1;
+  uint32_t k = 0;
+  uint32_t li = 0;
+  for (int item = blockIdx.x; item < nitems; item += gridDim.x, ++li) {
+    if (ob.pace)
+      while (*s_done < MMA_WARPS * (int)li) __nanosleep(256);
+    const int base = (item >> 1) * TC_M + (item & 1) * PREP_ROWS + (PREP_ROWS - ob.rows);
+    const int nrow = min(ob.rows, R - base);
+    uint32_t cur = 0;
+    if (nrow > 0 && lane < OBS_REC_W) cur = __ldg(ob.rec + (size_t)base * OBS_REC_W + lane);
+    for (int rl = 0; rl < nrow; ++rl) {
+      const size_t row = (size_t)(base + rl);
+      uint32_t nxt = 0;
+      if (rl + 1 < nrow && lane < OBS_REC_W) nxt = __ldg(ob.rec + (row + 1) * OBS_REC_W + lane);
+      const bool odd = k & 1;
+      float* rb = buf + (odd ? O : 0);
+      if (k >= 2) {
+        if (lane == 0) asm volatile("cp.async.bulk.wait_group.read 1;" ::: "memory");
+        __syncwarp();
+      }
+      const int old = odd ? set1 : set0;
+      if (old >= 0) rb[old] = 0.f;
+      int now = -1;
+      if (ob.tj) {
+        const bool live = __shfl_sync(IC3_FULL_MASK, cur, PREP_MAX_WW) != 0;
+        const float la = __uint_as_float(__shfl_sync(IC3_FULL_MASK, cur, PREP_MAX_WW + 1));
+        const float ri = __uint_as_float(__shfl_sync(IC3_FULL_MASK, cur, PREP_MAX_WW + 2));
+        if (lane < WW) {
+          const int c0 = 2 + lane * V, cls = (int)(cur & 0xffffu);
+          rb[c0 + ob.car_cls] = live ? (float)(cur >> 16) : 0.f;
+          if (live) {
+            rb[c0 + cls] = 1.f;
+            now = c0 + cls;
+          }
+        }
+        if (lane == 0) {
+          rb[0] = live ? la : 0.f;
+          rb[1] = live ? ri : 0.f;
+        }
+      } else if (lane < WW) {
+        const int c0 = lane * V, cls = (int)(cur & 0xffffu);
+        rb[c0 + V - 2] = (float)(cur >> 24);
+        rb[c0 + V - 1] = (float)((cur >> 16) & 0xffu);
+        rb[c0 + cls] = 1.f;
+        now = c0 + cls;
+      }
+      if (odd) set1 = now;
+      else set0 = now;
+      asm volatile("fence.proxy.async.shared::cta;" ::: "memory");
+      __syncwarp();
+      if (lane == 0) bulk_s2g(ob.obs + row * O, smem_u32(rb), (uint32_t)O * 4, !ob.keep);
+      cur = nxt;
+      ++k;
+    }
+  }
+  if (lane == 0) asm volatile("cp.async.bulk.wait_group 0;" ::: "memory");
+}
+
+constexpr int OBS_WARPS = 1;
+template <int OW>
+__global__ void __launch_bounds__(TC_P_THREADS + 32 * OW, 1) lstm_tc_kernel(ic3_policy_cfg cfg, ic3_policy_io io,
                                                                  const __half* __restrict__ a_img,
                                                                  const __half* __restrict__ b_img,
                                                                  const float* __restrict__ bias_cat, int nitems,
                                                                  const float* __restrict__ head_w, int nout,
-                                                                 float* __restrict__ partial) {
+                                                                 float* __restrict__ partial, ObsRows ob) {
   extern __shared__ __align__(1024) unsigned char smem[];
   uint64_t* bars = reinterpret_cast<uint64_t*>(smem + NSTAGE_P * STAGE_BYTES);
+  int* s_done = reinterpret_cast<int*>(smem + NSTAGE_P * STAGE_BYTES + 128);
   float* s_hw = reinterpret_cast<float*>(smem + NSTAGE_P * STAGE_BYTES + 256);
   float* s_bias = s_hw + TC_H * HEAD_PAD;
   ic3_pdl_trigger();
@@ -580,6 +716,7 @@
       mbar_init(bar_full + 8 * s, 1);
       mbar_init(bar_empty + 8 * s, MMA_WARPS);
     }
+    if (OW > 0) *s_done = 0;
     asm volatile("fence.mbarrier_init.release.cluster;" ::: "memory");
   }
   ic3_pdl_wait();
@@ -602,6 +739,8 @@
           [=](int item, int c) { return a + (size_t)(item >> 1) * TC_NCHUNK * A_CHUNK_BYTES + (size_t)c * (A_CHUNK_BYTES / 2); },
           [=](int item, int c) { return b + (size_t)((item & 1) * TC_NCHUNK + c) * B_CHUNK_BYTES; }, io.err);
     }
+  } else if (OW > 0 && warp > MMA_WARPS) {
+    lstm_obs_writer(ob, reinterpret_cast<float*>(smem + LSTM_SMEM_BYTES), s_done, cfg.B * cfg.N, nitems, lane);
   } else {
     const int wg = warp >> 2, w4 = warp & 3;
     float d[128];
@@ -612,6 +751,10 @@
     for (int item = blockIdx.x; item < nitems; item += gridDim.x, ++li) {
       wg_gemm_item<TC_NCHUNK>(d, smem_base, wg * 1024, bar_full, bar_empty, li, lane, ok, io.err);
       epilogue_item(cfg, io, s_bias, s_hw, partial, d, item >> 1, item & 1, wg, w4, lane, ok);
+      if (OW > 0) {
+        __syncwarp();
+        if (lane == 0) atomicAdd(s_done, 1);
+      }
     }
   }
 }
diff --git a/ic3net_b200/csrc/pp_env.cu b/ic3net_b200/csrc/pp_env.cu
--- a/ic3net_b200/csrc/pp_env.cu
+++ b/ic3net_b200/csrc/pp_env.cu
@@ -2,6 +2,7 @@
 
 #include "encoder_rows.cuh"
 #include "ic3_common.cuh"
+#include "obs_rows.cuh"
 #include "policy_internal.h"
 #include "rollout_tail.cuh"
 
@@ -71,36 +72,7 @@
   }
   __syncthreads();
   const int warp = threadIdx.x >> 5, lane = threadIdx.x & 31, nwarp = blockDim.x >> 5;
-  for (int c = warp; c < ncell; c += nwarp) {
-    const uint32_t info = s_cell[c];
-    const int cls = (int)(info & 0xffffu);
-    const float npred = (float)((info >> 16) & 0xffu), nprey = (float)(info >> 24);
-    float* dst = obs_env + (size_t)c * V;
-    if (VEC4) {
-      const int V4 = V >> 2, qc = cls >> 2, qp = (V - 1) >> 2, qy = (V - 2) >> 2;
-      for (int q = lane; q < V4; q += 32) {
-        float4 o = make_float4(0.f, 0.f, 0.f, 0.f);
-        if (q == qc) {
-          const int k = cls & 3;
-          o.x = k == 0 ? 1.f : 0.f; o.y = k == 1 ? 1.f : 0.f; o.z = k == 2 ? 1.f : 0.f; o.w = k == 3 ? 1.f : 0.f;
-        }
-        if (q == qy) {
-          o.z = nprey;
-        }
-        if (q == qp) {
-          o.w = npred;
-        }
-        ic3_st_obs(reinterpret_cast<float4*>(dst) + q, o, keep);
-      }
-    } else {
-      for (int q = lane; q < V; q += 32) {
-        float o = (q == cls) ? 1.f : 0.f;
-        if (q == V - 2) o = nprey;
-        if (q == V - 1) o = npred;
-        ic3_st_obs(dst + q, o, keep);
-      }
-    }
-  }
+  for (int c = warp; c < ncell; c += nwarp) pp_store_cell<VEC4>(s_cell[c], obs_env + (size_t)c * V, V, lane, keep);
 }
 
 template <bool VEC4>
diff --git a/ic3net_b200/csrc/tj_env.cu b/ic3net_b200/csrc/tj_env.cu
--- a/ic3net_b200/csrc/tj_env.cu
+++ b/ic3net_b200/csrc/tj_env.cu
@@ -2,6 +2,7 @@
 
 #include "encoder_rows.cuh"
 #include "ic3_common.cuh"
+#include "obs_rows.cuh"
 #include "policy_internal.h"
 #include "rollout_tail.cuh"
 
@@ -59,16 +60,7 @@
   const int warp = threadIdx.x >> 5, lane = threadIdx.x & 31, nwarp = blockDim.x >> 5;
   for (int c = warp; c < ncell; c += nwarp) {
     const int i = c / WW, w = c - i * WW;
-    const uint32_t info = s_cell[c];
-    const int cls = (int)(info & 0xffffu);
-    const float cnt = (float)(info >> 16);
-    const bool live = s_alive[i] != 0;
-    float* dst = obs_env + (size_t)i * O + 2 + (size_t)w * V;
-    for (int q = lane; q < V; q += 32) {
-      float o = (q == cls) ? 1.f : 0.f;
-      if (q == cfg.car_cls) o += cnt;
-      ic3_st_obs(dst + q, live ? o : 0.f, keep);
-    }
+    tj_store_cell(s_cell[c], s_alive[i] != 0, cfg.car_cls, obs_env + (size_t)i * O + 2 + (size_t)w * V, V, lane, keep);
   }
   for (int i = threadIdx.x; i < N; i += blockDim.x) {
     const bool live = s_alive[i] != 0;
diff --git a/ic3net_b200/trainer.py b/ic3net_b200/trainer.py
--- a/ic3net_b200/trainer.py
+++ b/ic3net_b200/trainer.py
@@ -69,7 +69,6 @@
         self._buf = None
         self._graph = None
         self._graph_key = None
-        self._side = None
         policy_net.set_obs_layout(*getattr(env.env, 'obs_layout', (0, 0, 0)))
         self.use_xtable = bool(getattr(args, 'encoder_table', True))
         self._xtable = None
@@ -177,6 +176,8 @@
         return (not dense) and self.policy_net.policy_impl == 'tc' and W * W <= 25
 
     OVERLAP_MIN_OBS_BYTES = 8 << 20
+    OBS_LSTM_ROWS = 64
+    OBS_LSTM_MIN_BYTES = 256 << 20
 
     def _overlap_obs(self):
         if self.obs_mode != 'dense' or (self.record_for_grad and self.is_tj and not self.grad_kernels):
@@ -203,17 +204,13 @@
         dense = self.obs_mode == 'dense' or (rec and self.is_tj and not gk)
         overlap = self._overlap_obs()
         fused_x = self._fused_x() or overlap
+        obs_bytes = B * N * self.env.observation_dim * 4
+        lstm_rows = self.OBS_LSTM_ROWS if obs_bytes >= self.OBS_LSTM_MIN_BYTES else 0
         src = {}
         if fused_x:
             src = dict(tj_env=C.addressof(e.cfg), tj_state=C.addressof(e.state)) if self.is_tj else \
                 dict(pp_env=C.addressof(e.cfg), pp_state=C.addressof(e.state))
             src['x_table'] = None if overlap else _lib.ptr(self._encoder_table(cfg, w))
-        if overlap:
-            main = torch.cuda.current_stream()
-            if self._side is None or self._side.device != main.device:
-                self._side = torch.cuda.Stream(device=main.device)
-            side = self._side
-            obs_write = lib.ic3_tj_obs_bounded if self.is_tj else lib.ic3_pp_obs_bounded
         fuse_heads = (net.policy_impl == 'tc' and 1 + sum(args.naction_heads) <= 8 and ws is not None
                       and bool(getattr(args, 'fuse_heads', False)))
         heads_kw = {}
@@ -247,11 +244,7 @@
                 if not gk and t % self.grad_window == 0:
                     b['ck_h'][t // self.grad_window].copy_(b['h'])
                     b['ck_c'][t // self.grad_window].copy_(b['c'])
-            if overlap:
-                side.wait_stream(main)
-                for ecfg, est, _, o_ptr, _ in self._dense_chunks(cfg):
-                    _lib.check(obs_write(C.byref(ecfg), C.byref(est), o_ptr, side.cuda_stream))
-            elif dense:
+            if dense and not overlap:
                 obs_enc = lib.ic3_tj_obs_encode if self.is_tj else lib.ic3_pp_obs_encode
                 for ecfg, est, ccfg, o_ptr, x_ptr in self._dense_chunks(cfg):
                     _lib.check(obs_enc(C.byref(ecfg), C.byref(est), C.byref(ccfg), C.byref(w), o_ptr, x_ptr, s))
@@ -272,12 +265,11 @@
                                fresh=b['fresh'].data_ptr(), tick=e.tick.data_ptr(), draws=None,
                                h_out=hout.data_ptr(), c_out=cout.data_ptr(), value=b['value'][t].data_ptr(),
                                logp=b['logp'][t].data_ptr(), action=b['action'][t].data_ptr(),
-                               workspace=_lib.ptr(ws), err=b['err'].data_ptr(), defer_heads=int(fuse_heads), **src)
+                               workspace=_lib.ptr(ws), err=b['err'].data_ptr(), defer_heads=int(fuse_heads),
+                               obs=b['obs'].data_ptr() if overlap else None, obs_lstm_rows=lstm_rows, **src)
             _lib.check(lib.ic3_policy_step(C.byref(cfg), C.byref(w), C.byref(io), s))
             if fuse_heads:
                 heads_kw.update(head_value=b['value'][t].data_ptr(), head_logp=b['logp'][t].data_ptr())
-            if overlap:
-                main.wait_stream(side)
             r = _lib.RolloutIO(t=t, max_steps=args.max_steps, nheads=nh, hard_attn=hard,
                                comm_action_one=int(bool(args.comm_action_one)),
                                last=int(t == T - 1 and quota <= 0), batch_size=int(quota),
diff --git a/include/ic3net_b200.h b/include/ic3net_b200.h
--- a/include/ic3net_b200.h
+++ b/include/ic3net_b200.h
@@ -235,6 +235,8 @@
   const float* x_table;
   int32_t defer_heads;
   int32_t pass_index;
+  float* obs;
+  int32_t obs_lstm_rows;
 } ic3_policy_io;
 
 const float* ic3_policy_partial_ptr(const ic3_policy_cfg* cfg, const void* workspace);
```

Measured after the change: 105.8 million (median of 6 runs). 1.05x the previous value.
